# KupynOrest/head_detector

Hardware: AMD Instinct MI355X
Metric: images/sec at 640x640 (VGGHeads forward path: net -> top-k/NMS -> FLAME decode) (higher is better)
Workload: dtype bf16; 1 GPU; vgg_heads_l bf16 batch 64/GPU @ 640x640, u8 NHWC input resident in HBM, ~2.88 heads/img decoded; one step = 8 forwards of that batch back to back (512 images per GPU per step); global_batch=64, image_size=640, parallelism=dp1, graph=False, exchange_to_rank0=False, overlap_post=True, batch_split=2, ramp_steps=30

## Files before the change

### head_detector_amd/csrc/detect.hip

```cpp
#include <hip/hip_runtime.h>

#include <cstring>
#include <new>
#include <vector>

#include "vgh_internal.h"

struct vgh_detector {
    vgh_net* net = nullptr;
    vgh_flame* flame = nullptr;
    vgh_detect_cfg cfg{};
    int device = 0, S = 0, arena_batch = 0, A = 0;
    float* boxes_all = nullptr;
    float* scores_all = nullptr;
    int32_t* idx = nullptr;
    float* cand_scores = nullptr;
    float* cand_boxes = nullptr;
    float* cand_flame = nullptr;
    int32_t* keep_idx = nullptr;
    int32_t* head_row = nullptr;
    int32_t* head_image = nullptr;
    int32_t* ticket = nullptr;
    bool lazy_flame = false;
    enum : uint8_t { SRC_NONE = 0, SRC_EAGER = 1, SRC_LAZY = 2 };
    std::vector<uint8_t> row_src;
    int lazy_rows = 0;
    uint64_t lazy_gen = 0;
    bool overlap = false, side_pending = false;
    hipStream_t side = nullptr, side_main = nullptr;
    bool side_low = true;
    bool side_own = false;
    hipEvent_t ev_net = nullptr, ev_cand = nullptr, ev_side = nullptr;
    vgh_lb_batch* lb = nullptr;
    const float* raw_unpad = nullptr;
};

namespace {

__global__ __launch_bounds__(1024) void head_list_kernel(const int32_t* __restrict__ counts, int B, int keep_k, int capacity, int32_t* __restrict__ head_row,
                                                        int32_t* __restrict__ head_image, int32_t* __restrict__ n_heads) {
    __shared__ int s_off[1025];
    const int t = threadIdx.x;
    const int per = (B + 1023) / 1024;
    const int b0 = t * per, b1 = min(B, b0 + per);
    int mine = 0;
    for (int b = b0; b < b1; ++b) mine += min(max(counts[b], 0), keep_k);
    s_off[t] = mine;
    __syncthreads();
    for (int d = 1; d < 1024; d <<= 1) {
        const int v = (t >= d) ? s_off[t - d] : 0;
        __syncthreads();
        s_off[t] += v;
        __syncthreads();
    }
    int at = s_off[t] - mine;
    if (t == 1023) *n_heads = min(s_off[1023], capacity);
    for (int b = b0; b < b1; ++b) {
        const int c = min(max(counts[b], 0), keep_k);
        for (int i = 0; i < c; ++i) {
            if (at + i < capacity) {
                head_row[at + i] = b * keep_k + i;
                head_image[at + i] = b;
            }
        }
        at += c;
    }
}

constexpr bool kSideLowPriority = true;

void release_side(vgh_detector* d) {
    if (!d->side) return;
    (void)hipStreamSynchronize(d->side);
    if (d->side_own)
        (void)hipStreamDestroy(d->side);
    else
        vgh_stream_release_internal(d->device, d->side, d->side_low);
    d->side = nullptr;
    d->side_own = false;
}

int ensure_side(vgh_detector* d, hipStream_t main) {
    if (d->side && d->side_main == main) return VGH_OK;
    hipStream_t avoid[4] = {main};
    if (int rc = vgh_net_lane_streams(d->net, main, avoid + 1)) return rc;
    release_side(d);
    if (int rc = vgh_stream_acquire_internal(d->device, avoid, 4, &d->side, d->side_low)) return rc;
    d->side_main = main;
    return VGH_OK;
}

}

extern "C" {

int vgh_detector_create(vgh_net* net, vgh_flame* flame, const vgh_detect_cfg* cfg, vgh_detector** out) {
    VGH_REQUIRE(net && cfg && out, "detector_create: null argument");
    VGH_REQUIRE(cfg->n_levels >= 1 && cfg->n_levels <= VGH_MAX_LEVELS, "detector_create: n_levels must be 1..%d", VGH_MAX_LEVELS);
    VGH_REQUIRE(cfg->pre_k >= 1 && cfg->pre_k <= 1024, "detector_create: pre_k must be 1..1024 (vgh_nms limit)");
    VGH_REQUIRE(cfg->keep_k >= 1 && cfg->keep_k <= cfg->pre_k, "detector_create: keep_k must be 1..pre_k");
    VGH_REQUIRE(cfg->max_batch >= 1, "detector_create: max_batch must be positive");
    VGH_REQUIRE(cfg->shape_live >= 0 && cfg->shape_live <= 300 && cfg->expr_live >= 0 && cfg->expr_live <= 100, "detector_create: live counts out of range");
    vgh_detector* d = new (std::nothrow) vgh_detector();
    VGH_REQUIRE(d, "detector_create: out of host memory");
    d->net = net;
    d->flame = flame;
    d->cfg = *cfg;
    d->S = vgh_net_image_size(net);
    d->device = vgh_net_device(net);
    d->arena_batch = vgh_net_max_batch(net);
    int A = 0;
    for (int l = 0; l < cfg->n_levels; ++l) {
        if (!vgh_net_buffer(net, cfg->level_buf[l])) {
            delete d;
            vgh_set_error("detector_create: level %d names buffer %d which the net does not have", l, cfg->level_buf[l]);
            return VGH_ERR_INVALID;
        }
        A += cfg->level_h[l] * cfg->level_w[l];
    }
    d->A = A;
    d->row_src.assign((size_t)cfg->max_batch, vgh_detector::SRC_NONE);
    if (cfg->pre_k > A) {
        delete d;
        vgh_set_error("detector_create: pre_k %d exceeds the %d anchors", cfg->pre_k, A);
        return VGH_ERR_INVALID;
    }
    const size_t MB = (size_t)cfg->max_batch, K = (size_t)cfg->pre_k, KK = (size_t)cfg->keep_k;
#define ALLOC(field, count)                                                           \
    if (hipMalloc((void**)&d->field, (count) * sizeof(*d->field)) != hipSuccess) {     \
        vgh_set_error("detector_create: hipMalloc(%s, %zu) failed", #field, (size_t)((count) * sizeof(*d->field))); \
        vgh_detector_destroy(d);                                                      \
        return VGH_ERR_NOMEM;                                                         \
    }
    ALLOC(boxes_all, MB * A * 4);
    ALLOC(scores_all, MB * A);
    ALLOC(idx, MB * K);
    ALLOC(cand_scores, MB * K);
    ALLOC(cand_boxes, MB * K * 4);
    ALLOC(cand_flame, MB * K * VGH_NUM_FLAME_PARAMS);
    ALLOC(keep_idx, MB * KK);
    ALLOC(head_row, MB * KK);
    ALLOC(head_image, MB * KK);
    ALLOC(ticket, 1);
#undef ALLOC
    if (hipMemset(d->ticket, 0, sizeof(int32_t)) != hipSuccess) {
        vgh_set_error("detector_create: hipMemset failed");
        vgh_detector_destroy(d);
        return VGH_ERR_HIP;
    }
    *out = d;
    return VGH_OK;
}

void vgh_detector_destroy(vgh_detector* d) {
    if (!d) return;
    hipFree(d->boxes_all);
    hipFree(d->scores_all);
    hipFree(d->idx);
    hipFree(d->cand_scores);
    hipFree(d->cand_boxes);
    hipFree(d->cand_flame);
    hipFree(d->keep_idx);
    hipFree(d->head_row);
    hipFree(d->head_image);
    hipFree(d->ticket);
    vgh_lb_destroy(d->lb);
    release_side(d);
    if (d->net) vgh_net_set_pred_guard(d->net, nullptr);
    if (d->ev_net) hipEventDestroy(d->ev_net);
    if (d->ev_cand) hipEventDestroy(d->ev_cand);
    if (d->ev_side) hipEventDestroy(d->ev_side);
    delete d;
}

int vgh_detector_candidates(vgh_detector* d, const void* images_dev, int image_fmt, int B, void* stream) {
    VGH_REQUIRE(d && images_dev, "detector_candidates: null argument");
    VGH_REQUIRE(B >= 1 && B <= d->cfg.max_batch, "detector_candidates: batch %d outside 1..%d", B, d->cfg.max_batch);
    VGH_REQUIRE(image_fmt == VGH_IMG_F32_NCHW || image_fmt == VGH_IMG_U8_NHWC || image_fmt == VGH_IMG_U8_RAW || image_fmt == VGH_IMG_YUV420_RAW,
                "detector_candidates: unknown image format %d", image_fmt);
    const bool raw = image_fmt == VGH_IMG_U8_RAW || image_fmt == VGH_IMG_YUV420_RAW;
    if (raw)
        if (int rc = vgh_lb_prepare(&d->lb, d->S, d->cfg.max_batch, d->arena_batch, image_fmt, images_dev, B)) return rc;
    const int fmt = raw ? VGH_IMG_U8_NHWC : image_fmt;
    const size_t img_bytes = (size_t)d->S * d->S * 3 * (fmt == VGH_IMG_F32_NCHW ? 4 : 1);
    const bool lazy = d->lazy_flame;
    if (B > d->arena_batch) d->lazy_flame = false;
    int rc = VGH_OK;
    for (int at = 0; at < B && !rc; at += d->arena_batch) {
        const int n = (B - at < d->arena_batch) ? B - at : d->arena_batch;
        const void* img = (const char*)images_dev + (size_t)at * img_bytes;
        if (raw) {
            rc = vgh_lb_chunk(d->lb, at / d->arena_batch, n, (hipStream_t)stream);
            img = vgh_lb_canvas(d->lb);
        }
        if (!rc) rc = vgh_net_forward(d->net, img, fmt, n, stream);
        if (!rc) rc = vgh_detector_decode_candidates(d, n, at, stream);
    }
    d->lazy_flame = lazy;
    d->raw_unpad = raw ? vgh_lb_unpad(d->lb) : nullptr;
    return rc;
}

int vgh_detector_decode_candidates(vgh_detector* d, int n, int at, void* stream) {
    VGH_REQUIRE(d, "detector_decode_candidates: null handle");
    VGH_REQUIRE(n >= 1 && at >= 0 && at + n <= d->cfg.max_batch && n <= d->arena_batch, "detector_decode_candidates: rows [%d,%d) outside the buffers", at, at + n);
    const vgh_detect_cfg& c = d->cfg;
    vgh_head_level lv[VGH_MAX_LEVELS];
    for (int l = 0; l < c.n_levels; ++l) {
        lv[l].pred_dev = (const float*)vgh_net_buffer(d->net, c.level_buf[l]);
        lv[l].h = c.level_h[l];
        lv[l].w = c.level_w[l];
        lv[l].pitch = c.level_pitch[l];
        lv[l].stride = c.level_stride[l];
    }
    void* st = stream;
    if (d->overlap) {
        if (int rc0 = ensure_side(d, (hipStream_t)stream)) return rc0;
        VGH_HIP(hipEventRecord(d->ev_net, (hipStream_t)stream));
        VGH_HIP(hipStreamWaitEvent(d->side, d->ev_net, 0));
        st = d->side;
    }
    float* ba = d->boxes_all + (size_t)at * d->A * 4;
    float* sa = d->scores_all + (size_t)at * d->A;
    int32_t* ix = d->idx + (size_t)at * c.pre_k;
    int rc;
    if ((rc = vgh_head_decode(lv, c.n_levels, n, ba, sa, st))) return rc;
    if ((rc = vgh_topk(sa, n, d->A, c.pre_k, ix, d->cand_scores + (size_t)at * c.pre_k, st))) return rc;
    const bool lazy = d->lazy_flame && at == 0;
    if ((rc = vgh_gather_candidates(lv, c.n_levels, n, d->A, c.shape_live, c.expr_live, ba, ix, c.pre_k, d->cand_boxes + (size_t)at * c.pre_k * 4,
                                    lazy ? nullptr : d->cand_flame + (size_t)at * c.pre_k * VGH_NUM_FLAME_PARAMS, st)))
        return rc;
    if (lazy) {
        for (int r = n; r < d->lazy_rows; ++r)
            if (d->row_src[r] == vgh_detector::SRC_LAZY) d->row_src[r] = vgh_detector::SRC_NONE;
        std::memset(d->row_src.data(), vgh_detector::SRC_LAZY, (size_t)n);
        d->lazy_rows = n;
        d->lazy_gen = vgh_net_generation(d->net);
    } else {
        std::memset(d->row_src.data() + at, vgh_detector::SRC_EAGER, (size_t)n);
    }
    if (d->overlap) {
        VGH_HIP(hipEventRecord(d->ev_cand, d->side));
        if ((rc = vgh_net_set_pred_guard(d->net, d->ev_cand))) return rc;
        d->side_pending = true;
    }
    return VGH_OK;
}

int vgh_detector_candidate_buffers(vgh_detector* d, float** boxes_dev, float** scores_dev, float** flame_dev) {
    VGH_REQUIRE(d, "detector_candidate_buffers: null handle");
    if (boxes_dev) *boxes_dev = d->cand_boxes;
    if (scores_dev) *scores_dev = d->cand_scores;
    if (flame_dev) *flame_dev = d->cand_flame;
    return VGH_OK;
}

void* vgh_detector_scratch(vgh_detector* d, int which) {
    if (!d) return nullptr;
    switch (which) {
        case VGH_SCRATCH_BOXES_ALL: return d->boxes_all;
        case VGH_SCRATCH_SCORES_ALL: return d->scores_all;
        case VGH_SCRATCH_TOPK_IDX: return d->idx;
        case VGH_SCRATCH_KEEP_IDX: return d->keep_idx;
        case VGH_SCRATCH_HEAD_ROW: return d->head_row;
        case VGH_SCRATCH_UNPAD: return vgh_lb_unpad(d->lb);
        case VGH_SCRATCH_CANVAS: return vgh_lb_canvas(d->lb);
        default: return nullptr;
    }
}

int vgh_detector_set_flame(vgh_detector* d, vgh_flame* flame) {
    VGH_REQUIRE(d, "detector_set_flame: null handle");
    d->flame = flame;
    return VGH_OK;
}

static int select_on(vgh_detector* d, int B, float conf_thr, float iou_thr, vgh_detect_out* o, void* stream) {
    const vgh_detect_cfg& c = d->cfg;
    int rc;
    const bool want_heads = o->proj_dev || o->verts_dev || o->rot_dev || o->rpy_dev || o->n_heads_dev || o->head_image_dev;
    VGH_REQUIRE(!want_heads || o->n_heads_dev, "detector_select: n_heads_dev is required when any per-head output is requested");
    const int cap_all = B * c.keep_k;
    const int capacity = (o->head_capacity > 0 && o->head_capacity < cap_all) ? o->head_capacity : cap_all;
    int32_t* himg = o->head_image_dev ? o->head_image_dev : d->head_image;
    int n_lazy = 0, n_none = 0;
    for (int r = 0; r < B; ++r) {
        n_lazy += d->row_src[r] == vgh_detector::SRC_LAZY;
        n_none += d->row_src[r] == vgh_detector::SRC_NONE;
    }
    VGH_REQUIRE(n_none == 0, "detector_select: %d of the candidate rows [0,%d) have no valid source (no candidate stage has filled them, or a shorter lazy one replaced theirs)", n_none, B);
    VGH_REQUIRE(n_lazy == 0 || n_lazy == B,
                "detector_select: rows [0,%d) mix %d lazily gathered rows with eagerly gathered ones; decode every chunk of such a batch with the lazy FLAME gather off", B, n_lazy);
    const bool lazy = n_lazy > 0;
    VGH_REQUIRE(!lazy || d->lazy_gen == vgh_net_generation(d->net),
                "detector_select: the candidates were gathered lazily from the predictions of forward %llu, but %llu forward(s) have been queued on the net since: the prediction "
                "buffers no longer hold that batch (queue the select before the next forward, or decode with the lazy FLAME gather off)",
                (unsigned long long)d->lazy_gen, (unsigned long long)(vgh_net_generation(d->net) - d->lazy_gen));
    VGH_REQUIRE(!lazy || c.keep_k <= 1024, "detector_select: the lazy FLAME gather needs keep_k <= 1024");
    if (c.keep_k <= 1024) {
        vgh_head_level lv[VGH_MAX_LEVELS];
        for (int l = 0; l < c.n_levels; ++l) {
            lv[l].pred_dev = (const float*)vgh_net_buffer(d->net, c.level_buf[l]);
            lv[l].h = c.level_h[l];
            lv[l].w = c.level_w[l];
            lv[l].pitch = c.level_pitch[l];
            lv[l].stride = c.level_stride[l];
        }
        if ((rc = vgh_nms_select(d->cand_boxes, d->cand_scores, d->cand_flame, B, c.pre_k, conf_thr, iou_thr, c.keep_k, d->keep_idx, o->counts_dev, o->boxes_dev,
                                 o->scores_dev, o->flame_dev, capacity, want_heads ? d->head_row : nullptr, himg, o->n_heads_dev, d->ticket, lazy ? lv : nullptr,
                                 c.n_levels, lazy ? d->idx : nullptr, c.shape_live, c.expr_live, stream)))
            return rc;
        if (lazy && d->overlap && stream == (void*)d->side) {
            VGH_HIP(hipEventRecord(d->ev_cand, d->side));
        }
        if (!want_heads) return VGH_OK;
    } else {
        if ((rc = vgh_nms(d->cand_boxes, d->cand_scores, B, c.pre_k, conf_thr, iou_thr, c.keep_k, d->keep_idx, o->counts_dev, stream))) return rc;
        if ((rc = vgh_compact(d->cand_boxes, d->cand_scores, d->cand_flame, B, c.pre_k, d->keep_idx, c.keep_k, o->boxes_dev, o->scores_dev, o->flame_dev, stream)))
            return rc;
        if (!want_heads) return VGH_OK;
        hipLaunchKernelGGL(head_list_kernel, dim3(1), dim3(1024), 0, (hipStream_t)stream, (const int32_t*)o->counts_dev, B, c.keep_k, capacity, d->head_row, himg,
                           o->n_heads_dev);
        VGH_HIP(hipGetLastError());
    }
    if (!(o->proj_dev || o->verts_dev || o->rot_dev || o->rpy_dev)) return VGH_OK;
    VGH_REQUIRE(d->flame, "detector_select: per-head FLAME outputs requested but the detector was created without a FLAME handle");
    const float* unpad = o->unpad_dev ? o->unpad_dev : d->raw_unpad;
    if ((rc = vgh_flame_decode_indirect(d->flame, o->flame_dev, d->head_row, himg, o->n_heads_dev, capacity, c.shape_live, c.expr_live, unpad, o->verts_dev,
                                        o->rot_dev, o->rpy_dev, o->proj_dev, stream)))
        return rc;
    return unpad && unpad == d->raw_unpad ? vgh_lb_unpad_read(d->lb, (hipStream_t)stream) : VGH_OK;
}

int vgh_detector_select(vgh_detector* d, int B, float conf_thr, float iou_thr, vgh_detect_out* o, void* stream) {
    VGH_REQUIRE(d && o, "detector_select: null argument");
    VGH_REQUIRE(B >= 1 && B <= d->cfg.max_batch, "detector_select: batch %d outside 1..%d", B, d->cfg.max_batch);
    VGH_REQUIRE(o->boxes_dev && o->scores_dev && o->flame_dev && o->counts_dev, "detector_select: boxes/scores/flame/counts outputs are mandatory");
    if (!d->overlap) return select_on(d, B, conf_thr, iou_thr, o, stream);
    if (int rc0 = ensure_side(d, (hipStream_t)stream)) return rc0;
    const int rc = select_on(d, B, conf_thr, iou_thr, o, d->side);
    d->side_pending = true;
    return rc;
}

#ifdef VGH_EXPERIMENTS
int vgh_detector_set_side_priority(vgh_detector* d, int low) {
    VGH_REQUIRE(d, "detector_set_side_priority: null handle");
    if ((low != 0) == d->side_low) return VGH_OK;
    if (d->side) VGH_HIP(hipStreamSynchronize(d->side));
    release_side(d);
    if (d->net) vgh_net_set_pred_guard(d->net, nullptr);
    d->side_pending = false;
    d->side_low = low != 0;
    return VGH_OK;
}
#endif

int vgh_detector_set_overlap(vgh_detector* d, int enable) {
    VGH_REQUIRE(d, "detector_set_overlap: null handle");
    if (enable && !d->ev_net) {
        VGH_HIP(hipEventCreateWithFlags(&d->ev_net, hipEventDisableTiming));
        VGH_HIP(hipEventCreateWithFlags(&d->ev_cand, hipEventDisableTiming));
        VGH_HIP(hipEventCreateWithFlags(&d->ev_side, hipEventDisableTiming));
    }
    if (!enable && d->side) {
        VGH_HIP(hipStreamSynchronize(d->side));
        vgh_net_set_pred_guard(d->net, nullptr);
        d->side_pending = false;
    }
    d->overlap = enable != 0;
    return VGH_OK;
}

int vgh_detector_set_lazy_flame(vgh_detector* d, int enable) {
    VGH_REQUIRE(d, "detector_set_lazy_flame: null handle");
    d->lazy_flame = enable != 0;
    return VGH_OK;
}

int vgh_detector_streams(vgh_detector* d, void* main_stream, void** out) {
    VGH_REQUIRE(d && out, "detector_streams: null argument");
    hipStream_t lanes[3];
    if (int rc = vgh_net_lane_streams(d->net, (hipStream_t)main_stream, lanes)) return rc;
    for (int i = 0; i < 3; ++i) out[i] = (void*)lanes[i];
    out[3] = nullptr;
    if (d->overlap) {
        if (int rc = ensure_side(d, (hipStream_t)main_stream)) return rc;
        out[3] = (void*)d->side;
    }
    return VGH_OK;
}

int vgh_detector_join(vgh_detector* d, void* stream) {
    VGH_REQUIRE(d, "detector_join: null handle");
    if (d->overlap && d->side && d->side_pending) {
        VGH_HIP(hipEventRecord(d->ev_side, d->side));
        VGH_HIP(hipStreamWaitEvent((hipStream_t)stream, d->ev_side, 0));
    }
    return VGH_OK;
}

int vgh_detector_record(vgh_detector* d, void* event, void* stream) {
    VGH_REQUIRE(d && event, "detector_record: null argument");
    if (d->overlap && d->side && d->side_pending)
        VGH_HIP(hipEventRecord((hipEvent_t)event, d->side));
    else
        VGH_HIP(hipEventRecord((hipEvent_t)event, (hipStream_t)stream));
    return VGH_OK;
}

int vgh_detect(vgh_detector* d, const void* images_dev, int image_fmt, int B, float conf_thr, float iou_thr, vgh_detect_out* o, void* stream) {
    int rc = vgh_detector_candidates(d, images_dev, image_fmt, B, stream);
    if (rc) return rc;
    return vgh_detector_select(d, B, conf_thr, iou_thr, o, stream);
}

}
```

### head_detector_amd/csrc/net.hip

```cpp
#include <stdarg.h>

#include <atomic>
#include <memory>
#include <vector>

#include "net_plan.h"
#include "per_device.h"
#include "vgh_internal.h"

static thread_local char g_err[1024] = "";

void vgh_set_error(const char* fmt, ...) {
    va_list ap;
    va_start(ap, fmt);
    vsnprintf(g_err, sizeof(g_err), fmt, ap);
    va_end(ap);
}

struct NetOp {
    vgh_op_desc d;
    uint16_t* wpack = nullptr;
    float* wf32 = nullptr;
    float* bias = nullptr;
    float out_scale = 1.0f;
    int auto_cfg = -1;
    uint16_t* wds = nullptr;
    float* gscale = nullptr;
    float* dvec = nullptr;
    int overhang_ok = 0, b2b = 0;
    hipEvent_t ev_done = nullptr;
};

static std::atomic<int> g_i8_diag{1};

struct vgh_net {
    int device = 0, image_size = 0, max_batch = 0;
    std::vector<vgh_buf_desc> bufs;
    std::vector<void*> buf_ptr;
    std::vector<int64_t> buf_bytes;
    std::vector<NetOp> ops;
    char* arena = nullptr;
    char* wblob = nullptr;
    uint16_t* zeros = nullptr;
    hipGraph_t graph = nullptr;
    hipGraphExec_t graph_exec = nullptr;
    static constexpr int kLanes = kNetLanes;
    hipStream_t side[kLanes] = {nullptr, nullptr, nullptr, nullptr};
    hipStream_t lanes_main = nullptr;
    bool lanes_ready = false;
    hipEvent_t ev_fork = nullptr, ev_join[kLanes] = {nullptr, nullptr, nullptr, nullptr}, ev_lag[kLanes] = {nullptr, nullptr, nullptr, nullptr};
    hipEvent_t pred_guard = nullptr;
    int nsplit = 1;
    int stem_pair = -1;
    bool lane_wait_cycle = false;
    int fuse_b2b = 1;
    int stem3_ok = 0;
    uint64_t generation = 0;
    int fuse_stem = 0;
};

static inline int64_t buf_image_bytes(const vgh_buf_desc& b) { return (int64_t)b.h * b.w * b.pitch * vgh_fmt_bytes(b.is_f32); }
static inline char* buf_at(const vgh_net* n, int id, int at) { return (char*)n->buf_ptr[id] + at * buf_image_bytes(n->bufs[id]); }

static int net_conv_args(vgh_net* n, const NetOp& op, int B, int at, ConvArgs* a) {
    const vgh_op_desc& d = op.d;
    const vgh_buf_desc &ib = n->bufs[d.in_buf], &ob = n->bufs[d.out_buf];
    const vgh_buf_desc* rb = d.res_buf >= 0 ? &n->bufs[d.res_buf] : nullptr;
    conv_args_fill(a, d, ConvGeom{ib.is_f32, ob.is_f32 == VGH_FMT_F32, vgh_fmt_q8_kind(ob.is_f32), B, ib.h, ib.w, ib.pitch, ob.pitch, rb ? rb->pitch : 0, vgh_fmt_planes(ob.is_f32), rb ? vgh_fmt_planes(rb->is_f32) : 0});
    a->in = (const uint16_t*)buf_at(n, d.in_buf, at);
    a->out = buf_at(n, d.out_buf, at);
    a->res = rb ? (const uint16_t*)buf_at(n, d.res_buf, at) : nullptr;
    a->wpack = op.wpack;
    a->bias = op.bias;
    a->gscale = op.gscale;
    a->dvec = op.dvec;
    a->out_scale = op.out_scale;
    a->zeros = n->zeros;
    const bool in8 = vgh_fmt_is_q8(ib.is_f32), out8 = vgh_fmt_is_q8(ob.is_f32);
    VGH_REQUIRE(a->out_f32 || ob.is_f32 == ib.is_f32 || (in8 && ob.is_f32 == VGH_FMT_BF16) || (out8 && ib.is_f32 == VGH_FMT_BF16), "net: op writes buffer %d in another format than it reads", d.out_buf);
    VGH_REQUIRE(!rb || rb->is_f32 == (in8 ? VGH_FMT_BF16 : ib.is_f32), "net: residual buffer %d has another format than the input", d.res_buf);
    VGH_REQUIRE(!(in8 || out8) || (d.ksize == 3 && d.stride == 1 && !d.grp_cout && !d.shuffle && (!in8 || d.cin % 64 == 0)), "net: an e4m3 buffer can only link plain 3x3 / stride-1 convs (cin %% 64 == 0)");
    const int eh = d.shuffle ? 2 * a->Ho : a->Ho, ew = d.shuffle ? 2 * a->Wo : a->Wo;
    VGH_REQUIRE(ob.h == eh && ob.w == ew, "net: op output buffer %d is %dx%d, conv produces %dx%d", d.out_buf, ob.h, ob.w, eh, ew);
    VGH_REQUIRE(op.overhang_ok || d.in_coff + d.cin + (d.grp_cout ? (d.cout_pad / d.grp_cout - 1) * d.grp_in_stride : 0) <= ib.pitch, "net: conv reads past the input pitch (buf %d)", d.in_buf);
    return VGH_OK;
}

static void net_b2b_fields(ConvArgs& a, const ConvArgs& a2) {
    a.w2pack = a2.wpack;
    a.bias2 = a2.bias;
    a.out2 = a2.out;
    a.out2_pitch = a2.out_pitch;
    a.out2_coff = a2.out_coff;
    a.out2_coff2 = a2.out_coff2;
    a.out2_split = a2.out_split;
    a.cout2_pad = a2.cout_pad;
    a.cout2_store = a2.cout_store;
    a.act2 = a2.act;
}

static bool stem_in_pair_launch(const vgh_net* n) { return n->fuse_b2b == 1 && n->stem_pair >= 0 && n->stem3_ok == 1 && n->ops[n->stem_pair + 1].b2b == 1; }

static int net_run_op(vgh_net* n, const NetOp& op, const void* image0, int fmt, int B, int at, hipStream_t st, int share = 1) {
    const vgh_op_desc& d = op.d;
    const void* image = (const char*)image0 + (int64_t)at * n->image_size * n->image_size * 3 * (fmt == VGH_IMG_F32_NCHW ? 4 : 1);
    const int op_index = (int)(&op - n->ops.data());
    const bool fused = n->fuse_stem && n->stem_pair >= 0;
    const bool stem3 = stem_in_pair_launch(n) && !fused && fmt == VGH_IMG_U8_NHWC;
    switch (d.kind) {
        case VGH_OP_STEM: {
            if (stem3 && op_index == n->stem_pair) {
                const NetOp &ds = n->ops[op_index + 1], &nx = n->ops[op_index + 2];
                ConvArgs a, a2;
                if (int rc = net_conv_args(n, ds, B, at, &a)) return rc;
                if (int rc = net_conv_args(n, nx, B, at, &a2)) return rc;
                a.grid_share = share;
                net_b2b_fields(a, a2);
                return vgh_launch_stem_ds_b2b(a, image, n->image_size, n->image_size, op.wf32, op.bias, st);
            }
#ifdef VGH_EXPERIMENTS
            if (fused && op_index == n->stem_pair) {
                const NetOp& ds = n->ops[op_index + 1];
                const vgh_buf_desc& db = n->bufs[ds.d.out_buf];
                return vgh_launch_stem_ds(image, fmt, B, n->image_size, n->image_size, op.wf32, op.bias, ds.wds, ds.bias, (uint16_t*)buf_at(n, ds.d.out_buf, at), db.pitch, ds.d.out_coff, st);
            }
#endif
            const vgh_buf_desc& ob = n->bufs[d.out_buf];
            if (ob.is_f32 == VGH_FMT_F32)
                return vgh_launch_stem_f32(image, fmt, B, n->image_size, n->image_size, op.wf32, op.bias, (float*)buf_at(n, d.out_buf, at), ob.pitch, d.out_coff, st);
            if (ob.is_f32 == VGH_FMT_F16)
                return vgh_launch_stem(image, fmt, B, n->image_size, n->image_size, op.wf32, op.bias, (uint16_t*)buf_at(n, d.out_buf, at), ob.pitch, d.out_coff, d.cout_store, VGH_FMT_F16X2, 0, st);
            return vgh_launch_stem(image, fmt, B, n->image_size, n->image_size, op.wf32, op.bias, (uint16_t*)buf_at(n, d.out_buf, at), (int64_t)ob.pitch * vgh_fmt_planes(ob.is_f32), d.out_coff,
                                   d.cout_store, ob.is_f32, ob.pitch, st);
        }
        case VGH_OP_CONV: {
            if ((fused || stem3) && op_index == n->stem_pair + 1) return VGH_OK;
            if (n->fuse_b2b && op.b2b == 2) return VGH_OK;
            ConvArgs a;
            if (int rc = net_conv_args(n, op, B, at, &a)) return rc;
            a.grid_share = share;
            if (n->fuse_b2b && op.b2b == 1) {
                const NetOp& nx = n->ops[op_index + 1];
                ConvArgs a2;
                if (int rc = net_conv_args(n, nx, B, at, &a2)) return rc;
                net_b2b_fields(a, a2);
                a.b2b_igemm = n->fuse_b2b == 2;
                return vgh_launch_conv_b2b(a, st);
            }
            if (n->bufs[d.in_buf].is_f32 != VGH_FMT_F32) {
                a.fallback_cfg1 = op.auto_cfg + 1;
                return vgh_launch_conv(a, d.force_cfg >= 0 ? d.force_cfg : op.auto_cfg, st);
            }
            VGH_REQUIRE(a.out_f32 && (d.res_buf < 0 || n->bufs[d.res_buf].is_f32 == VGH_FMT_F32), "net: fp32 conv needs fp32 output / residual buffers");
            VGH_REQUIRE(!d.grp_cout, "net: the fp32 FMA kernel has no grouped mode");
            return vgh_launch_conv_f32(a, op.wf32, st);
        }
        case VGH_OP_SPP_POOL: {
            const vgh_buf_desc& ib = n->bufs[d.in_buf];
            if (ib.is_f32 == VGH_FMT_F32) return vgh_launch_spp_pool_f32((float*)buf_at(n, d.in_buf, at), ib.pitch, d.in_coff, d.cin, B, ib.h, ib.w, st);
            if (ib.is_f32 == VGH_FMT_F16) return vgh_launch_spp_pool((uint16_t*)buf_at(n, d.in_buf, at), ib.pitch, d.in_coff, d.cin, B, ib.h, ib.w, VGH_FMT_F16X2, 0, st);
            return vgh_launch_spp_pool((uint16_t*)buf_at(n, d.in_buf, at), (int64_t)ib.pitch * vgh_fmt_planes(ib.is_f32), d.in_coff, d.cin, B, ib.h, ib.w, ib.is_f32, ib.pitch, st);
        }
        case VGH_OP_FORK:
            return VGH_OK;
        default:
            VGH_REQUIRE(false, "net: unknown op kind %d", d.kind);
    }
    return VGH_OK;
}

static int ensure_lanes(vgh_net* n, hipStream_t main) {
    if (n->lanes_ready && n->lanes_main == main) return VGH_OK;
    hipStreamCaptureStatus cs = hipStreamCaptureStatusNone;
    if (hipStreamIsCapturing(main, &cs) == hipSuccess && cs != hipStreamCaptureStatusNone) {
        VGH_REQUIRE(n->lanes_ready, "net: the lane streams cannot be picked while the caller's stream is capturing; run vgh_net_capture (or one forward) first");
        return VGH_OK;
    }
    hipStream_t avoid[vgh_net::kLanes] = {main};
    for (int l = 1; l < vgh_net::kLanes; ++l) {
        if (n->side[l]) {
            VGH_HIP(hipStreamSynchronize(n->side[l]));
            vgh_stream_release_internal(n->device, n->side[l]);
            n->side[l] = nullptr;
        }
    }
    for (int l = 1; l < vgh_net::kLanes; ++l) {
        if (int rc = vgh_stream_acquire_internal(n->device, avoid, l, &n->side[l])) return rc;
        avoid[l] = n->side[l];
    }
    n->lanes_main = main;
    n->lanes_ready = true;
    return VGH_OK;
}

int vgh_net_lane_streams(vgh_net* n, hipStream_t main, hipStream_t* out) {
    if (int rc = ensure_lanes(n, main)) return rc;
    for (int l = 1; l < vgh_net::kLanes; ++l) out[l - 1] = n->side[l];
    return VGH_OK;
}

static std::atomic<int> g_lane_lag{0};

static int net_forward_split(vgh_net* n, const void* image_dev, int image_fmt, int B, hipStream_t main) {
    const int L = n->nsplit < B ? n->nsplit : B;
    int at[vgh_net::kLanes + 1];
    at[0] = 0;
    for (int l = 0; l < L; ++l) at[l + 1] = at[l] + rows_of_lane(B, L, l);
    VGH_HIP(hipEventRecord(n->ev_fork, main));
    for (int l = 1; l < L; ++l) VGH_HIP(hipStreamWaitEvent(n->side[l], n->ev_fork, 0));
    std::vector<const NetOp*> seq;
    seq.reserve(n->ops.size());
    for (const NetOp& op : n->ops)
        if (op.d.kind != VGH_OP_FORK) seq.push_back(&op);
    const int N = (int)seq.size();
    int lag = g_lane_lag.load(std::memory_order_relaxed);
    if (lag < 0) lag = 0;
    if (lag > N) lag = N;
    bool guard_pending[vgh_net::kLanes];
    for (int l = 0; l < L; ++l) guard_pending[l] = n->pred_guard != nullptr;
    for (int s = 0; s < N + lag * (L - 1); ++s) {
        for (int l = 0; l < L; ++l) {
            const int i = s - l * lag;
            if (i < 0 || i >= N) continue;
            const NetOp& op = *seq[i];
            hipStream_t st = l == 0 ? main : n->side[l];
            if (lag > 0 && l > 0 && i == 0) VGH_HIP(hipStreamWaitEvent(st, n->ev_lag[l - 1], 0));
            if (guard_pending[l] && op.d.kind == VGH_OP_CONV && n->bufs[op.d.out_buf].is_f32 == VGH_FMT_F32) {
                VGH_HIP(hipStreamWaitEvent(st, n->pred_guard, 0));
                guard_pending[l] = false;
            }
            if (int rc = net_run_op(n, op, image_dev, image_fmt, at[l + 1] - at[l], at[l], st)) return rc;
            if (lag > 0 && l + 1 < L && i == lag - 1) VGH_HIP(hipEventRecord(n->ev_lag[l], st));
        }
    }
    for (int l = 1; l < L; ++l) {
        VGH_HIP(hipEventRecord(n->ev_join[l], n->side[l]));
        VGH_HIP(hipStreamWaitEvent(main, n->ev_join[l], 0));
    }
    return VGH_OK;
}

static void pack_weights(const NetPlan& plan, const vgh_buf_desc* bufs, const vgh_op_desc* ops, int n_ops, const float* weights_host, const float* biases_host, char* host, float* oscale) {
#ifdef VGH_EXPERIMENTS
    if (plan.stem_pair >= 0) vgh_pack_stem_ds_weights_host(weights_host + ops[plan.stem_pair + 1].w_off, (uint16_t*)(host + plan.wds));
#endif
    for (int i = 0; i < n_ops; ++i) {
        const vgh_op_desc& d = ops[i];
        const NetPlan::Op& po = plan.ops[i];
        if (d.kind == VGH_OP_CONV) {
            const int wf = bufs[d.in_buf].is_f32;
            if (wf == VGH_FMT_F32)
                memcpy(host + po.w, weights_host + d.w_off, (size_t)d.cout_pad * d.ksize * d.ksize * d.cin * 4);
            else if (wf == VGH_FMT_BF16)
                vgh_pack_conv_weights_host(weights_host + d.w_off, d.cout_pad, d.ksize, d.cin, (uint16_t*)(host + po.w));
            else if (vgh_fmt_is_q8(wf))
                ;
            else
                vgh_pack_conv_weights_split_host(weights_host + d.w_off, d.cout_pad, d.ksize, d.cin, wf, (uint16_t*)(host + po.w), &oscale[i]);
            memcpy(host + po.bias, biases_host + d.b_off, (size_t)d.cout_pad * 4);
            if (po.gscale >= 0) {
                float* g = (float*)(host + po.gscale);
                float* bq = (float*)(host + po.bias);
                const float s_out = vgh_fmt_is_q8(bufs[d.out_buf].is_f32) ? bufs[d.out_buf].scale : 1.0f;
                if (wf == VGH_FMT_I8) {
                    std::vector<float> ws(d.cout_pad);
                    const float* wsrc = weights_host + d.w_off;
                    std::vector<float> peeled;
                    if (po.dvec >= 0) {
                        peeled.assign(wsrc, wsrc + (size_t)d.cout_pad * 9 * d.cin);
                        float* dv = (float*)(host + po.dvec);
                        for (int c = 0; c < d.cout_pad; ++c) {
                            float& wd = peeled[(size_t)c * 9 * d.cin + (size_t)4 * d.cin + c];
                            dv[c] = wd * bufs[d.in_buf].scale;
                            wd = 0.0f;
                        }
                        wsrc = peeled.data();
                    }
                    vgh_pack_conv_weights_i8_host(wsrc, d.cout_pad, d.ksize, d.cin, (uint8_t*)(host + po.w), ws.data());
                    for (int c = 0; c < d.cout_pad; ++c) {
                        const float acc_unit = ws[c] * bufs[d.in_buf].scale;
                        g[c] = acc_unit / s_out;
                        const float bi = __builtin_nearbyintf(bq[c] / acc_unit);
                        const int32_t b32 = bi != bi ? 0 : bi > 2.0e9f ? 2000000000 : bi < -2.0e9f ? -2000000000 : (int32_t)bi;
                        memcpy(&bq[c], &b32, 4);
                    }
                } else if (wf == VGH_FMT_FP8) {
                    std::vector<float> ws(d.cout_pad);
                    vgh_pack_conv_weights_fp8_host(weights_host + d.w_off, d.cout_pad, d.ksize, d.cin, (uint8_t*)(host + po.w), ws.data());
                    for (int c = 0; c < d.cout_pad; ++c) {
                        const float acc_unit = ws[c] * bufs[d.in_buf].scale;
                        bq[c] = bq[c] / acc_unit;
                        g[c] = acc_unit / s_out;
                    }
                } else {
                    for (int c = 0; c < d.cout_pad; ++c) g[c] = 1.0f / s_out;
                }
            }
        } else if (d.kind == VGH_OP_STEM) {
            float* dst = (float*)(host + po.w);
            for (int co = 0; co < 48; ++co)
                for (int k = 0; k < 27; ++k) dst[k * 48 + co] = weights_host[d.w_off + co * 27 + k];
            memcpy(host + po.bias, biases_host + d.b_off, 48 * 4);
        }
    }
}

static int require_canvas(const char* who, int image_fmt) {
    VGH_REQUIRE(image_fmt == VGH_IMG_F32_NCHW || image_fmt == VGH_IMG_U8_NHWC, "%s: image format %d is not a canvas (VGH_IMG_U8_RAW and VGH_IMG_YUV420_RAW are letterboxed by vgh_detect)", who, image_fmt);
    return VGH_OK;
}

struct NetDestroy {
    void operator()(vgh_net* net) const { vgh_net_destroy(net); }
};

extern "C" {

const char* vgh_version(void) { return "vgh 0.1.0 (gfx950)"; }
const char* vgh_last_error(void) { return g_err; }
int vgh_abi_version(void) { return VGH_ABI_VERSION; }

int vgh_net_create(int device, int image_size, int max_batch, const vgh_buf_desc* bufs, int n_bufs, const vgh_op_desc* ops, int n_ops,
                   const float* weights_host, int64_t n_weights, const float* biases_host, int64_t n_biases, vgh_net** out) {
    VGH_REQUIRE(out && bufs && ops && weights_host && biases_host, "net_create: null argument");
    VGH_REQUIRE(max_batch >= 1 && image_size >= 32 && image_size % 32 == 0, "net_create: bad max_batch / image_size");
    NetPlan plan;
    if (int rc = net_plan(image_size, max_batch, bufs, n_bufs, ops, n_ops, weights_host, n_weights, n_biases, g_i8_diag.load(std::memory_order_relaxed) != 0, &plan)) {
        vgh_set_error("%s", plan.err);
        return rc;
    }
    VGH_HIP(hipSetDevice(device));
    std::unique_ptr<vgh_net, NetDestroy> guard(new vgh_net());
    vgh_net* n = guard.get();
    n->device = device;
    n->image_size = image_size;
    n->max_batch = max_batch;
    n->bufs.assign(bufs, bufs + n_bufs);
    n->buf_bytes = plan.buf_bytes;
    n->stem_pair = plan.stem_pair;
    n->lane_wait_cycle = plan.lane_wait_cycle;
    VGH_HIP(hipMalloc((void**)&n->arena, plan.arena_bytes));
    VGH_HIP(hipMemset(n->arena, 0, plan.arena_bytes));
    for (int i = 0; i < n_bufs; ++i) n->buf_ptr.push_back(n->arena + plan.buf_off[i]);
    VGH_HIP(hipMalloc((void**)&n->zeros, 256));
    VGH_HIP(hipMemset(n->zeros, 0, 256));
    VGH_HIP(hipEventCreateWithFlags(&n->ev_fork, hipEventDisableTiming));
    for (int l = 1; l < vgh_net::kLanes; ++l) VGH_HIP(hipEventCreateWithFlags(&n->ev_join[l], hipEventDisableTiming));
    for (int l = 0; l < vgh_net::kLanes; ++l) VGH_HIP(hipEventCreateWithFlags(&n->ev_lag[l], hipEventDisableTiming));
    std::vector<char> host(plan.blob_bytes > 0 ? plan.blob_bytes : 1, 0);
    std::vector<float> oscale(n_ops, 1.0f);
    pack_weights(plan, bufs, ops, n_ops, weights_host, biases_host, host.data(), oscale.data());
    VGH_HIP(hipMalloc((void**)&n->wblob, host.size()));
    VGH_HIP(hipMemcpy(n->wblob, host.data(), host.size(), hipMemcpyHostToDevice));
    for (int i = 0; i < n_ops; ++i) {
        const NetPlan::Op& po = plan.ops[i];
        NetOp op;
        op.d = ops[i];
        op.out_scale = oscale[i];
        op.overhang_ok = po.overhang_ok;
        op.b2b = po.b2b;
        if (ops[i].kind == VGH_OP_CONV || ops[i].kind == VGH_OP_STEM) {
            op.wf32 = (float*)(n->wblob + po.w);
            op.bias = (float*)(n->wblob + po.bias);
        }
        if (ops[i].kind == VGH_OP_CONV) op.wpack = (uint16_t*)(n->wblob + po.w);
        if (po.gscale >= 0) op.gscale = (float*)(n->wblob + po.gscale);
        if (po.dvec >= 0) op.dvec = (float*)(n->wblob + po.dvec);
        if (plan.wds >= 0 && i == plan.stem_pair + 1) op.wds = (uint16_t*)(n->wblob + plan.wds);
        n->ops.push_back(op);
        if (po.ev_done) VGH_HIP(hipEventCreateWithFlags(&n->ops[i].ev_done, hipEventDisableTiming));
    }
    for (NetOp& op : n->ops) {
        if (op.d.kind != VGH_OP_CONV || n->bufs[op.d.in_buf].is_f32 == VGH_FMT_F32) continue;
        ConvArgs ref;
        if (int rc = net_conv_args(n, op, n->max_batch, 0, &ref)) return rc;
        if (int rc = vgh_conv_prepare(ref)) return rc;
        op.auto_cfg = vgh_conv_pick_auto(ref);
    }
    if (n->stem_pair >= 0 && n->stem_pair + 2 < (int)n->ops.size() && n->ops[n->stem_pair + 1].b2b == 1 && image_size % 32 == 0) {
        ConvArgs a, a2;
        if (!net_conv_args(n, n->ops[n->stem_pair + 1], 1, 0, &a) && !net_conv_args(n, n->ops[n->stem_pair + 2], 1, 0, &a2)) {
            net_b2b_fields(a, a2);
            if (!vgh_conv_prepare(a)) n->stem3_ok = vgh_conv_ds_b2b_ok(a) && a.act == VGH_ACT_RELU ? 1 : 0;
        }
    }
    *out = guard.release();
    return VGH_OK;
}

void vgh_net_destroy(vgh_net* n) {
    if (!n) return;
    if (n->graph_exec) hipGraphExecDestroy(n->graph_exec);
    if (n->graph) hipGraphDestroy(n->graph);
    for (int l = 1; l < vgh_net::kLanes; ++l) {
        if (n->side[l]) {
            hipStreamSynchronize(n->side[l]);
            vgh_stream_release_internal(n->device, n->side[l]);
        }
        if (n->ev_join[l]) hipEventDestroy(n->ev_join[l]);
    }
    for (int l = 0; l < vgh_net::kLanes; ++l)
        if (n->ev_lag[l]) hipEventDestroy(n->ev_lag[l]);
    if (n->ev_fork) hipEventDestroy(n->ev_fork);
    for (NetOp& op : n->ops)
        if (op.ev_done) hipEventDestroy(op.ev_done);
    hipFree(n->arena);
    hipFree(n->wblob);
    hipFree(n->zeros);
    delete n;
}

int vgh_net_forward(vgh_net* n, const void* image_dev, int image_fmt, int B, void* stream) {
    VGH_REQUIRE(n && image_dev, "net_forward: null argument");
    if (int rc = require_canvas("net_forward", image_fmt)) return rc;
    VGH_REQUIRE(B >= 0 && B <= n->max_batch, "net_forward: B=%d exceeds max_batch=%d", B, n->max_batch);
    hipStream_t main = (hipStream_t)stream;
    ++n->generation;
    if (int rc = ensure_lanes(n, main)) return rc;
    if (n->nsplit > 1 && B > 1) return net_forward_split(n, image_dev, image_fmt, B, main);
    bool pending[vgh_net::kLanes] = {false, false, false, false}, used[vgh_net::kLanes] = {false, false, false, false};
    bool guard_pending = n->pred_guard != nullptr;
    for (const NetOp& op : n->ops) {
        if (guard_pending && op.d.kind == VGH_OP_CONV && n->bufs[op.d.out_buf].is_f32 == VGH_FMT_F32) {
            VGH_HIP(hipStreamWaitEvent(main, n->pred_guard, 0));
            for (int l = 1; l < vgh_net::kLanes; ++l)
                if (n->side[l]) VGH_HIP(hipStreamWaitEvent(n->side[l], n->pred_guard, 0));
            guard_pending = false;
        }
        if (op.d.kind == VGH_OP_FORK) {
            VGH_HIP(hipEventRecord(n->ev_fork, main));
            for (int l = 1; l < vgh_net::kLanes; ++l) pending[l] = true;
            continue;
        }
        const int lane_f = op.d.lane & 0xff, dep = (op.d.lane >> 8) - 1;
        const int lane = (lane_f > 0 && lane_f < vgh_net::kLanes) ? lane_f : 0;
        hipStream_t st = main;
        if (lane > 0) {
            st = n->side[lane];
            if (pending[lane]) {
                VGH_HIP(hipStreamWaitEvent(st, n->ev_fork, 0));
                pending[lane] = false;
            }
            used[lane] = true;
        }
        if (dep >= 0 && dep < (int)n->ops.size() && n->ops[dep].ev_done) VGH_HIP(hipStreamWaitEvent(st, n->ops[dep].ev_done, 0));
        if (int rc = net_run_op(n, op, image_dev, image_fmt, B, 0, st)) return rc;
        if (op.ev_done) VGH_HIP(hipEventRecord(op.ev_done, st));
    }
    for (int l = 1; l < vgh_net::kLanes; ++l)
        if (used[l]) {
            VGH_HIP(hipEventRecord(n->ev_join[l], n->side[l]));
            VGH_HIP(hipStreamWaitEvent(main, n->ev_join[l], 0));
        }
    return VGH_OK;
}

int vgh_net_profile(vgh_net* n, const void* image_dev, int image_fmt, int B, void* stream, float* op_ms) {
    VGH_REQUIRE(n && image_dev && op_ms, "net_profile: null argument");
    if (int rc = require_canvas("net_profile", image_fmt)) return rc;
    VGH_REQUIRE(B >= 0 && B <= n->max_batch, "net_profile: B=%d exceeds max_batch=%d", B, n->max_batch);
    hipStream_t st = (hipStream_t)stream;
    ++n->generation;
    if (int rc = ensure_lanes(n, st)) return rc;
    const size_t m = n->ops.size();
    struct Events {
        std::vector<hipEvent_t> v;
        ~Events() {
            for (hipEvent_t e : v)
                if (e) hipEventDestroy(e);
        }
    } events{std::vector<hipEvent_t>(m + 1, nullptr)};
    std::vector<hipEvent_t>& ev = events.v;
    for (auto& e : ev) VGH_HIP(hipEventCreate(&e));
    VGH_HIP(hipEventRecord(ev[0], st));
    const int L = (n->nsplit > 1 && B > 1) ? (n->nsplit < B ? n->nsplit : B) : 1;
    for (size_t i = 0; i < m; ++i) {
        if (L == 1) {
            if (int rc = net_run_op(n, n->ops[i], image_dev, image_fmt, B, 0, st)) return rc;
        } else {
            VGH_HIP(hipEventRecord(n->ev_fork, st));
            int at = 0;
            for (int l = 0; l < L; ++l) {
                const int nb = rows_of_lane(B, L, l);
                hipStream_t ls = l == 0 ? st : n->side[l];
                if (l > 0) VGH_HIP(hipStreamWaitEvent(ls, n->ev_fork, 0));
                if (int rc = net_run_op(n, n->ops[i], image_dev, image_fmt, nb, at, ls)) return rc;
                if (l > 0) {
                    VGH_HIP(hipEventRecord(n->ev_join[l], ls));
                    VGH_HIP(hipStreamWaitEvent(st, n->ev_join[l], 0));
                }
                at += nb;
            }
        }
        VGH_HIP(hipEventRecord(ev[i + 1], st));
    }
    VGH_HIP(hipEventSynchronize(ev[m]));
    for (size_t i = 0; i < m; ++i) VGH_HIP(hipEventElapsedTime(&op_ms[i], ev[i], ev[i + 1]));
    return VGH_OK;
}

int vgh_net_capture(vgh_net* n, const void* image_dev, int image_fmt, int B, void* stream) {
    VGH_REQUIRE(n && stream, "net_capture: needs a non-null stream");
    if (int rc = require_canvas("net_capture", image_fmt)) return rc;
    VGH_REQUIRE(!n->pred_guard, "net_capture: a prediction guard event is set (detector overlap mode); graph replay cannot honour it");
    VGH_REQUIRE(!n->lane_wait_cycle, "net_capture: two side lanes of this program wait for each other's ops; the HIP runtime cannot end the capture of such a program (run it eagerly, "
                "or lay the lanes out so that the wait-for relation among lanes 1..3 is acyclic, as arch.schedule_latency does)");
    hipStream_t st = (hipStream_t)stream;
    if (n->graph_exec) {
        hipGraphExecDestroy(n->graph_exec);
        n->graph_exec = nullptr;
    }
    if (n->graph) {
        hipGraphDestroy(n->graph);
        n->graph = nullptr;
    }
    if (int rc = ensure_lanes(n, st)) return rc;
    VGH_HIP(hipStreamBeginCapture(st, hipStreamCaptureModeThreadLocal));
    int rc = vgh_net_forward(n, image_dev, image_fmt, B, stream);
    hipError_t e = hipStreamEndCapture(st, &n->graph);
    if (rc) return rc;
    VGH_HIP(e);
    VGH_HIP(hipGraphInstantiate(&n->graph_exec, n->graph, nullptr, nullptr, 0));
    return VGH_OK;
}

int vgh_net_forward_graph(vgh_net* n, void* stream) {
    VGH_REQUIRE(n && n->graph_exec, "net_forward_graph: call vgh_net_capture first");
    VGH_REQUIRE(!n->pred_guard, "net_forward_graph: a prediction guard event is set (detector overlap mode); use vgh_net_forward");
    ++n->generation;
    VGH_HIP(hipGraphLaunch(n->graph_exec, (hipStream_t)stream));
    return VGH_OK;
}

void* vgh_net_buffer(vgh_net* n, int buf_id) { return (n && buf_id >= 0 && buf_id < (int)n->buf_ptr.size()) ? n->buf_ptr[buf_id] : nullptr; }
int64_t vgh_net_buffer_bytes(vgh_net* n, int buf_id) { return (n && buf_id >= 0 && buf_id < (int)n->buf_bytes.size()) ? n->buf_bytes[buf_id] : -1; }

#ifdef VGH_EXPERIMENTS
int vgh_net_set_lane_lag(int ops) {
    VGH_REQUIRE(ops >= 0, "net_set_lane_lag: negative");
    g_lane_lag.store(ops, std::memory_order_relaxed);
    return VGH_OK;
}
#endif

int vgh_net_set_split(vgh_net* n, int nsplit) {
    VGH_REQUIRE(n, "net_set_split: null handle");
    VGH_REQUIRE(nsplit >= 1 && nsplit <= vgh_net::kLanes, "net_set_split: 1..%d lanes", vgh_net::kLanes);
    n->nsplit = nsplit;
    return VGH_OK;
}

#ifdef VGH_EXPERIMENTS
int vgh_net_set_fuse_stem(vgh_net* n, int enable) {
    VGH_REQUIRE(n, "net_set_fuse_stem: null handle");
    n->fuse_stem = enable ? 1 : 0;
    return VGH_OK;
}
#endif

int vgh_net_set_pred_guard(vgh_net* n, void* event) {
    VGH_REQUIRE(n, "net_set_pred_guard: null handle");
    n->pred_guard = (hipEvent_t)event;
    return VGH_OK;
}

int vgh_net_set_b2b(vgh_net* n, int enable) {
    VGH_REQUIRE(n, "net_set_b2b: null handle");
    n->fuse_b2b = (enable == 2 || enable == 3) ? enable : enable ? 1 : 0;
    return VGH_OK;
}
int vgh_net_stem_fused(vgh_net* n) {
    return n && stem_in_pair_launch(n) ? 1 : 0;
}
int vgh_net_b2b_pairs(vgh_net* n) {
    int k = 0;
    if (n)
        for (const NetOp& op : n->ops) k += op.b2b == 1;
    return k;
}

uint64_t vgh_net_generation(vgh_net* n) { return n ? n->generation : 0; }
int vgh_net_max_batch(vgh_net* n) { return n ? n->max_batch : 0; }
int vgh_net_device(vgh_net* n) { return n ? n->device : 0; }
int vgh_net_image_size(vgh_net* n) { return n ? n->image_size : 0; }

int vgh_net_set_cfg(vgh_net* n, int op_index, int cfg) {
    VGH_REQUIRE(n && op_index >= 0 && op_index < (int)n->ops.size(), "net_set_cfg: bad op index");
    const int fmt0 = n->bufs[n->ops[op_index].d.kind == VGH_OP_CONV ? n->ops[op_index].d.in_buf : 0].is_f32;
    const bool split_net = vgh_fmt_planes(fmt0) > 1 || fmt0 == VGH_FMT_F16;
    VGH_REQUIRE(cfg >= -1 && cfg < (split_net ? vgh_conv_split_num_cfgs() : vgh_conv_num_cfgs()), "net_set_cfg: bad cfg");
    NetOp& op = n->ops[op_index];
    if (cfg >= 0 && op.d.kind == VGH_OP_CONV && !split_net && (n->bufs[op.d.in_buf].is_f32 == VGH_FMT_BF16 || vgh_fmt_is_q8(n->bufs[op.d.in_buf].is_f32))) {
        ConvArgs ref;
        int rc = net_conv_args(n, op, n->max_batch, 0, &ref);
        if (!rc) rc = vgh_conv_prepare(ref);
        if (rc) return rc;
        if (!vgh_conv_cfg_ok_for(cfg, ref)) {
            fprintf(stderr, "[vgh] net_set_cfg: op %d: tile %s cannot run this op at max_batch=%d; its automatic tile %s runs it at every batch size\n", op_index, vgh_conv_cfg_name(cfg),
                    n->max_batch, vgh_conv_cfg_name(op.auto_cfg));
            cfg = -1;
        }
    }
    op.d.force_cfg = cfg;
    return VGH_OK;
}

int vgh_net_op_cfg(vgh_net* n, int op_index) {
    if (!n || op_index < 0 || op_index >= (int)n->ops.size()) return -1;
    const NetOp& op = n->ops[op_index];
    if (op.d.kind != VGH_OP_CONV || n->bufs[op.d.in_buf].is_f32 == VGH_FMT_F32) return -1;
    return op.d.force_cfg >= 0 ? op.d.force_cfg : op.auto_cfg;
}

static uint16_t* g_zeros[kMaxDevices];
static PerDevice g_zeros_made;

int vgh_conv2d(const vgh_conv_call* c, void* stream) {
    VGH_REQUIRE(c && c->in_dev && c->wpack_dev && c->bias_dev && c->out_dev, "conv2d: null argument");
    int dev = 0;
    VGH_HIP(hipGetDevice(&dev));
    VGH_REQUIRE(device_slot(hipSuccess, dev) != kNoSlot, "conv2d: device index");
    hipError_t zeros_err = hipSuccess;
    once_per_device(g_zeros_made, dev, [&] {
        uint16_t* z = nullptr;
        if ((zeros_err = hipMalloc((void**)&z, 256)) == hipSuccess && (zeros_err = hipMemset(z, 0, 256)) == hipSuccess) g_zeros[dev] = z;
        return zeros_err == hipSuccess ? 1 : 0;
    });
    VGH_HIP(zeros_err);
    VGH_REQUIRE(c->fmt == VGH_FMT_BF16 || c->fmt == VGH_FMT_BF16X2 || c->fmt == VGH_FMT_F16X2 || c->fmt == VGH_FMT_FP8 || c->fmt == VGH_FMT_F16 || c->fmt == VGH_FMT_I8, "conv2d: fmt %d", c->fmt);
    const int in_fp8 = vgh_fmt_q8_kind(c->fmt);
    VGH_REQUIRE(c->out_fp8 >= 0 && c->out_fp8 <= 2 && (!in_fp8 || !c->out_fp8 || in_fp8 == c->out_fp8), "conv2d: out_fp8 is 0, 1 (e4m3) or 2 (int8), and an 8-bit input keeps its format");
    VGH_REQUIRE(!c->diag_dev || (c->fmt == VGH_FMT_I8 && !c->out_fp8 && c->cin >= c->cout_pad && c->cout_pad <= 1024), "conv2d: diag_dev belongs to an int8 -> bf16 conv with cout_pad <= min(cin, 1024)");
    VGH_REQUIRE(!(in_fp8 || c->out_fp8) || (c->gscale_dev && (vgh_fmt_is_q8(c->fmt) || c->fmt == VGH_FMT_BF16) && !c->out_f32), "conv2d: an e4m3 / int8 conv needs gscale_dev, a bf16 or e4m3 input and no fp32 output");
    const int planes = vgh_fmt_planes(c->fmt);
    ConvArgs a;
    conv_args_fill(&a, *c, ConvGeom{c->fmt, c->out_f32, c->out_fp8, c->B, c->H, c->W, c->in_pitch, c->out_pitch, c->res_pitch, c->out_f32 ? 1 : planes, planes});
    a.in = (const uint16_t*)c->in_dev;
    a.out = c->out_dev;
    a.res = (const uint16_t*)c->res_dev;
    a.wpack = (const uint16_t*)c->wpack_dev;
    a.bias = c->bias_dev;
    a.gscale = c->gscale_dev;
    a.dvec = c->diag_dev;
    a.out_scale = c->out_scale;
    a.zeros = g_zeros[dev];
    return vgh_launch_conv(a, c->force_cfg, (hipStream_t)stream);
}

int vgh_pack_conv_weights(const float* w_host, int cout_pad, int ksize, int cin, uint16_t* wpack_host) {
    VGH_REQUIRE(w_host && wpack_host, "pack: null argument");
    VGH_REQUIRE(cin % 32 == 0 && cout_pad % 32 == 0 && (ksize == 1 || ksize == 3), "pack: cin/cout_pad must be multiples of 32, ksize 1 or 3");
    vgh_pack_conv_weights_host(w_host, cout_pad, ksize, cin, wpack_host);
    return VGH_OK;
}

int vgh_pack_conv_weights_fp8(const float* w_host, int cout_pad, int ksize, int cin, uint8_t* wpack_host, float* wscale_host) {
    VGH_REQUIRE(w_host && wpack_host && wscale_host, "pack_fp8: null argument");
    VGH_REQUIRE(cin % 64 == 0 && cout_pad % 32 == 0 && ksize == 3, "pack_fp8: cin must be a multiple of 64, cout_pad of 32, ksize 3");
    vgh_pack_conv_weights_fp8_host(w_host, cout_pad, ksize, cin, wpack_host, wscale_host);
    return VGH_OK;
}
int vgh_net_set_i8_diag(int on) {
    g_i8_diag.store(on ? 1 : 0, std::memory_order_relaxed);
    return VGH_OK;
}
int vgh_net_op_has_diag(vgh_net* n, int op_index) { return (n && op_index >= 0 && op_index < (int)n->ops.size() && n->ops[op_index].dvec) ? 1 : 0; }
int vgh_pack_conv_weights_i8(const float* w_host, int cout_pad, int ksize, int cin, uint8_t* wpack_host, float* wscale_host) {
    VGH_REQUIRE(w_host && wpack_host && wscale_host, "pack_i8: null argument");
    VGH_REQUIRE(cin % 64 == 0 && cout_pad % 32 == 0 && ksize == 3, "pack_i8: cin must be a multiple of 64, cout_pad of 32, ksize 3");
    vgh_pack_conv_weights_i8_host(w_host, cout_pad, ksize, cin, wpack_host, wscale_host);
    return VGH_OK;
}

int vgh_stream_create(int device, void** stream_out) {
    VGH_REQUIRE(stream_out, "stream_create: null");
    VGH_HIP(hipSetDevice(device));
    hipStream_t s;
    VGH_HIP(hipStreamCreateWithFlags(&s, hipStreamNonBlocking));
    *stream_out = (void*)s;
    return VGH_OK;
}
int vgh_stream_destroy(void* stream) {
    VGH_HIP(hipStreamDestroy((hipStream_t)stream));
    return VGH_OK;
}
int vgh_stream_sync(void* stream) {
    VGH_HIP(hipStreamSynchronize((hipStream_t)stream));
    return VGH_OK;
}
int vgh_event_create(void** ev_out) {
    VGH_REQUIRE(ev_out, "event_create: null");
    hipEvent_t e;
    VGH_HIP(hipEventCreate(&e));
    *ev_out = (void*)e;
    return VGH_OK;
}
int vgh_event_destroy(void* ev) {
    VGH_HIP(hipEventDestroy((hipEvent_t)ev));
    return VGH_OK;
}
int vgh_event_record(void* ev, void* stream) {
    VGH_HIP(hipEventRecord((hipEvent_t)ev, (hipStream_t)stream));
    return VGH_OK;
}
int vgh_event_elapsed_ms(void* ev_start, void* ev_stop, float* ms_out) {
    VGH_REQUIRE(ms_out, "event_elapsed: null");
    VGH_HIP(hipEventSynchronize((hipEvent_t)ev_stop));
    VGH_HIP(hipEventElapsedTime(ms_out, (hipEvent_t)ev_start, (hipEvent_t)ev_stop));
    return VGH_OK;
}

}
```

### head_detector_amd/csrc/net_plan.h

```cpp
#pragma once
#include <math.h>
#include <stdint.h>
#include <stdio.h>
#include <string.h>

#include <vector>

#include "../../include/vgh.h"
#include "conv_tiles.h"

constexpr int kNetLanes = 4;

inline int64_t align_up(int64_t x, int64_t a) { return (x + a - 1) / a * a; }

inline int rows_of_lane(int B, int L, int l) { return B / L + (l < B % L ? 1 : 0); }

struct ConvGeom {
    int fmt;
    int out_f32, out_fp8;
    int B, H, W;
    int64_t in_pitch, out_pitch, res_pitch;
    int out_planes, res_planes;
};
template <class Desc>
inline void conv_args_fill(ConvArgs* a, const Desc& d, const ConvGeom& g) {
    memset(a, 0, sizeof(*a));
    const bool h16 = g.fmt == VGH_FMT_F16;
    a->split = h16 ? VGH_FMT_F16X2 : vgh_fmt_planes(g.fmt) > 1 ? g.fmt : 0;
    a->nseg = h16 ? 1 : 3;
    a->in_plane = h16 ? 0 : (int)g.in_pitch;
    a->out_plane = h16 ? 0 : (int)g.out_pitch;
    a->res_plane = h16 ? 0 : (int)g.res_pitch;
    a->grp_cout = d.grp_cout;
    a->grp_in_stride = d.grp_in_stride;
    a->in_pitch = g.in_pitch * vgh_fmt_planes(g.fmt);
    a->in_coff = d.in_coff;
    a->cin = d.cin;
    a->B = g.B;
    a->H = g.H;
    a->W = g.W;
    a->ksize = d.ksize;
    a->stride = d.stride;
    a->pad = d.ksize / 2;
    a->Ho = (g.H + 2 * a->pad - d.ksize) / d.stride + 1;
    a->Wo = (g.W + 2 * a->pad - d.ksize) / d.stride + 1;
    a->out_pitch = g.out_pitch * g.out_planes;
    a->out_coff = d.out_coff;
    a->out_coff2 = d.out_coff2;
    a->out_split = d.out_split;
    a->cout_pad = d.cout_pad;
    a->cout_store = d.cout_store;
    a->out_f32 = g.out_f32;
    a->res_pitch = g.res_pitch * g.res_planes;
    a->res_coff = d.res_coff;
    a->in_fp8 = vgh_fmt_q8_kind(g.fmt);
    a->out_fp8 = g.out_fp8;
    a->alpha = d.alpha;
    a->act = d.act;
    a->shuffle = d.shuffle;
    a->shuffle_c = d.shuffle ? d.cout_pad / 4 : 0;
    a->P = g.B * a->Ho * a->Wo;
    a->cblocks = d.cin / (a->in_fp8 ? 64 : 32);
    a->nkb = d.ksize * d.ksize * a->cblocks;
}

inline bool i8_peel_diag(const float* w, const vgh_op_desc& d, bool enabled) {
    if (!enabled || d.ksize != 3 || d.stride != 1 || d.grp_cout || d.cin < d.cout_pad || d.cout_pad > 1024) return false;
    const size_t row = (size_t)9 * d.cin;
    int live = 0, dom = 0;
    for (int c = 0; c < d.cout_pad; ++c) {
        float mx = 0.0f;
        for (size_t i = 0; i < row; ++i) mx = fmaxf(mx, fabsf(w[(size_t)c * row + i]));
        if (mx > 0.0f) {
            ++live;
            if (fabsf(w[(size_t)c * row + (size_t)4 * d.cin + c]) >= mx) ++dom;
        }
    }
    return live > 0 && 2 * dom >= live;
}

inline bool sole_link(const vgh_op_desc* ops, int n_ops, int i, int buf) {
    for (int j = 0; j < n_ops; ++j)
        if (j != i && j != i + 1 && (ops[j].kind == VGH_OP_CONV || ops[j].kind == VGH_OP_SPP_POOL) && (ops[j].in_buf == buf || ops[j].out_buf == buf || ops[j].res_buf == buf)) return false;
    return true;
}

struct NetPlan {
    std::vector<int64_t> buf_off, buf_bytes;
    int64_t arena_bytes = 0;
    struct Op {
        int64_t w = 0, bias = 0;
        int64_t gscale = -1;
        int64_t dvec = -1;
        int b2b = 0;
        int overhang_ok = 0;
        int ev_done = 0;
    };
    std::vector<Op> ops;
    int64_t wds = -1;
    int64_t blob_bytes = 0;
    int stem_pair = -1;
    bool lane_wait_cycle = false;
    char err[256] = "";
};

inline int net_plan(int image_size, int max_batch, const vgh_buf_desc* bufs, int n_bufs, const vgh_op_desc* ops, int n_ops, const float* weights, int64_t n_weights, int64_t n_biases,
                    bool i8_diag, NetPlan* p) {
#define PLAN_REQUIRE(cond, ...)                          \
    do {                                                 \
        if (!(cond)) {                                   \
            snprintf(p->err, sizeof(p->err), __VA_ARGS__); \
            return VGH_ERR_INVALID;                      \
        }                                                \
    } while (0)
    *p = NetPlan();
    PLAN_REQUIRE(n_bufs >= 0 && n_ops >= 0, "net_create: negative buffer or op count");
    for (int i = 0; i < n_bufs; ++i) {
        PLAN_REQUIRE(bufs[i].is_f32 >= VGH_FMT_BF16 && bufs[i].is_f32 <= VGH_FMT_I8, "net_create: buffer %d has unknown format %d", i, bufs[i].is_f32);
        PLAN_REQUIRE(!vgh_fmt_is_q8(bufs[i].is_f32) || (bufs[i].scale > 0.0f && bufs[i].scale < 1e30f && bufs[i].pitch % 16 == 0), "net_create: 8-bit buffer %d needs a positive scale and a pitch that is a multiple of 16", i);
        const int64_t bytes = (int64_t)max_batch * bufs[i].h * bufs[i].w * bufs[i].pitch * vgh_fmt_bytes(bufs[i].is_f32);
        p->buf_off.push_back(p->arena_bytes);
        p->buf_bytes.push_back(bytes);
        p->arena_bytes += align_up(bytes + 256, 256);
    }
    const auto buf_ok = [&](int id) { return id >= 0 && id < n_bufs; };
    p->ops.assign(n_ops, NetPlan::Op());
    int64_t at = 0;
    const auto take = [&](int64_t bytes) {
        const int64_t off = at;
        at += align_up(bytes, 256);
        return off;
    };
    for (int i = 0; i < n_ops; ++i) {
        const vgh_op_desc& d = ops[i];
        NetPlan::Op& o = p->ops[i];
        if (d.kind == VGH_OP_CONV) {
            PLAN_REQUIRE(d.cin % 32 == 0 && d.cout_pad % 32 == 0, "net_create: op %d channel padding", i);
            PLAN_REQUIRE(buf_ok(d.in_buf) && buf_ok(d.out_buf) && d.res_buf < n_bufs, "net_create: op %d buffer ids", i);
            const int64_t we = (int64_t)d.cout_pad * d.ksize * d.ksize * d.cin;
            PLAN_REQUIRE(d.w_off >= 0 && d.w_off + we <= n_weights && d.b_off >= 0 && d.b_off + d.cout_pad <= n_biases, "net_create: op %d weight range", i);
            const vgh_buf_desc& ib = bufs[d.in_buf];
            if (d.in_coff + d.cin > ib.pitch && !d.grp_cout) {
                const int live = ib.pitch - d.in_coff;
                PLAN_REQUIRE(live > 0 && ib.is_f32 == VGH_FMT_BF16, "net_create: op %d reads past the pitch of buffer %d", i, d.in_buf);
                const float* w = weights + d.w_off;
                for (int64_t r = 0; r < (int64_t)d.cout_pad * d.ksize * d.ksize; ++r)
                    for (int c = live; c < d.cin; ++c)
                        PLAN_REQUIRE(w[r * d.cin + c] == 0.0f, "net_create: op %d reads %d channels of a %d-channel pitch with a non-zero weight at input channel %d", i, d.cin, ib.pitch, c);
                o.overhang_ok = 1;
            }
            const int wf = ib.is_f32, of = bufs[d.out_buf].is_f32;
            o.w = take(we * (vgh_fmt_is_q8(wf) ? 1 : (wf == VGH_FMT_BF16 || wf == VGH_FMT_F16) ? 2 : wf == VGH_FMT_F32 ? 4 : 6));
            o.bias = take((int64_t)d.cout_pad * 4);
            if (vgh_fmt_is_q8(wf) || vgh_fmt_is_q8(of)) {
                o.gscale = take((int64_t)d.cout_pad * 4);
                if (wf == VGH_FMT_I8 && of == VGH_FMT_BF16 && i8_peel_diag(weights + d.w_off, d, i8_diag)) o.dvec = take((int64_t)d.cout_pad * 4);
            }
        } else if (d.kind == VGH_OP_STEM) {
            PLAN_REQUIRE(buf_ok(d.out_buf), "net_create: op %d buffer ids", i);
            PLAN_REQUIRE(d.w_off >= 0 && d.w_off + 27 * 48 <= n_weights && d.b_off >= 0 && d.b_off + 48 <= n_biases, "net_create: stem weight range");
            o.w = take(27 * 48 * 4);
            o.bias = take(64 * 4);
        } else if (d.kind == VGH_OP_SPP_POOL) {
            PLAN_REQUIRE(buf_ok(d.in_buf), "net_create: op %d buffer ids", i);
        }
        if (d.lane >> 8) {
            const int dep = (d.lane >> 8) - 1;
            PLAN_REQUIRE(dep >= 0 && dep < i, "net_create: op %d waits for op %d, which does not precede it", i, dep);
            p->ops[dep].ev_done = 1;
        }
    }
    for (int i = 0; i + 1 < n_ops; ++i) {
        const vgh_op_desc &a = ops[i], &d = ops[i + 1];
        if (a.kind != VGH_OP_STEM || d.kind != VGH_OP_CONV) continue;
        if (image_size % 4 == 0  && d.in_buf == a.out_buf && d.in_coff == a.out_coff && d.ksize == 3 && d.stride == 2 && d.cin == 64 &&
            d.cout_pad == 96 && d.cout_store == 96 && d.res_buf < 0 && !d.shuffle && d.out_split >= 96 && d.act == VGH_ACT_RELU && d.grp_cout == 0 && bufs[a.out_buf].is_f32 == VGH_FMT_BF16 &&
            bufs[d.out_buf].is_f32 == VGH_FMT_BF16 && d.out_coff % 8 == 0 && bufs[d.out_buf].pitch % 8 == 0 && sole_link(ops, n_ops, i, a.out_buf)) {
            p->stem_pair = i;
#ifdef VGH_EXPERIMENTS
            p->wds = take((int64_t)9 * 3 * 96 * 16 * 2);
#endif
        }
        break;
    }
    p->blob_bytes = at;
    for (int i = 0; i + 1 < n_ops; ++i) {
        const vgh_op_desc &a = ops[i], &b = ops[i + 1];
        if (a.kind != VGH_OP_CONV || b.kind != VGH_OP_CONV || p->ops[i].b2b != 0) continue;
        const vgh_buf_desc &ab = bufs[a.out_buf], &ai = bufs[a.in_buf], &bo = bufs[b.out_buf];
        if (ab.is_f32 == VGH_FMT_BF16 && ai.is_f32 == VGH_FMT_BF16 && bo.is_f32 == VGH_FMT_BF16 && vgh_conv_b2b_ok(a.ksize, a.stride, a.cout_pad, b.cout_pad) && a.cout_store == a.cout_pad &&
            a.out_coff == 0 && a.out_split >= a.cout_pad && ab.pitch == a.cout_pad && a.res_buf < 0 && !a.shuffle && !a.grp_cout && a.act != VGH_ACT_SILU && b.ksize == 1 && b.stride == 1 &&
            b.in_buf == a.out_buf && b.in_coff == 0 && b.cin == a.cout_pad && b.res_buf < 0 && !b.shuffle && !b.grp_cout && b.act != VGH_ACT_SILU && b.out_coff % 8 == 0 && b.out_coff2 % 8 == 0 &&
            b.out_split % 8 == 0 && b.cout_store % 8 == 0 && bo.pitch % 8 == 0 && sole_link(ops, n_ops, i, a.out_buf)) {
            p->ops[i].b2b = 1;
            p->ops[i + 1].b2b = 2;
        }
    }
    bool w[kNetLanes][kNetLanes] = {};
    for (int i = 0; i < n_ops; ++i) {
        if (!(ops[i].lane >> 8)) continue;
        const int a = ops[i].lane & 0xff, b = ops[(ops[i].lane >> 8) - 1].lane & 0xff;
        if (a > 0 && a < kNetLanes && b > 0 && b < kNetLanes && a != b) w[a][b] = true;
    }
    for (int k = 1; k < kNetLanes; ++k)
        for (int a = 1; a < kNetLanes; ++a)
            for (int b = 1; b < kNetLanes; ++b) w[a][b] = w[a][b] || (w[a][k] && w[k][b]);
    for (int a = 1; a < kNetLanes; ++a) p->lane_wait_cycle = p->lane_wait_cycle || w[a][a];
    return VGH_OK;
#undef PLAN_REQUIRE
}
```

### head_detector_amd/csrc/postproc.hip

```cpp
#include "vgh_internal.h"

namespace {

constexpr int MAX_LEVELS = 4;
struct Levels {
    const float* pred[MAX_LEVELS];
    int h[MAX_LEVELS], w[MAX_LEVELS], pitch[MAX_LEVELS], stride[MAX_LEVELS], start[MAX_LEVELS + 1];
    int n;
};

__device__ __forceinline__ int find_level(const Levels& L, int a) {
    int l = 0;
#pragma unroll
    for (int i = 1; i < MAX_LEVELS; ++i)
        if (i < L.n && a >= L.start[i]) l = i;
    return l;
}

__global__ __launch_bounds__(256) void head_decode_kernel(Levels L, int B, int A, float* __restrict__ boxes, float* __restrict__ scores) {
    const int64_t gid = (int64_t)blockIdx.x * blockDim.x + threadIdx.x;
    if (gid >= (int64_t)B * A) return;
    const int b = (int)(gid / A), a = (int)(gid - (int64_t)b * A);
    const int l = find_level(L, a);
    const int p = a - L.start[l];
    const int hw = L.h[l] * L.w[l];
    const float* pr = L.pred[l] + ((int64_t)b * hw + p) * L.pitch[l];
    const int ay = p / L.w[l], ax = p - ay * L.w[l];
    float d[4];
#pragma unroll
    for (int side = 0; side < 4; ++side) {
        float x[17];
        float m = -INFINITY;
#pragma unroll
        for (int k = 0; k < 17; ++k) {
            x[k] = pr[side * 17 + k];
            m = fmaxf(m, x[k]);
        }
        float s = 0.0f;
#pragma unroll
        for (int k = 0; k < 17; ++k) {
            x[k] = expf(x[k] - m);
            s += x[k];
        }
        float e = 0.0f;
#pragma unroll
        for (int k = 0; k < 17; ++k) e += (x[k] / s) * (float)k;
        d[side] = e;
    }
    const float cx = (float)ax + 0.5f, cy = (float)ay + 0.5f, st = (float)L.stride[l];
    float4 o;
    o.x = (cx - d[0]) * st;
    o.y = (cy - d[1]) * st;
    o.z = (cx + d[2]) * st;
    o.w = (cy + d[3]) * st;
    *(float4*)(boxes + gid * 4) = o;
    scores[gid] = 1.0f / (1.0f + expf(-pr[VGH_PRED_CLS_OFF]));
}

__device__ __forceinline__ uint32_t float_key(float f) {
    uint32_t u = __float_as_uint(f);
    if ((u & 0x7fffffffu) > 0x7f800000u) return 0xffffffffu;
    if (u == 0x80000000u) u = 0u;
    return (u & 0x80000000u) ? ~u : (u | 0x80000000u);
}
template <bool FILTER>
__device__ __forceinline__ uint64_t composite(float f, int idx, float conf) {
    const uint32_t key = (FILTER && !(f >= conf)) ? 0u : float_key(f);
    return ((uint64_t)key << 32) | (uint32_t)(~(uint32_t)idx);
}

template <bool CACHED, bool FILTER>
__global__ __launch_bounds__(1024) void topk_kernel(const float* __restrict__ scores, int A, int k, int32_t* __restrict__ out_idx,
                                                    float* __restrict__ out_scores, float conf) {
    constexpr int RC = 9;
    __shared__ uint32_t hist[256];
    __shared__ uint64_t s_prefix;
    __shared__ int s_kk;
    __shared__ int s_count;
    __shared__ int s_done;
    __shared__ uint64_t sel[1024];
    const int b = blockIdx.x, tid = threadIdx.x;
    const float* sc = scores + (int64_t)b * A;
    if (tid == 0) {
        s_prefix = 0;
        s_kk = k;
        s_count = 0;
        s_done = 0;
    }
    sel[tid] = 0;
    uint64_t cache[RC];
    if constexpr (CACHED) {
#pragma unroll
        for (int r = 0; r < RC; ++r) {
            const int i = tid + r * 1024;
            cache[r] = i < A ? composite<FILTER>(sc[i], i, conf) : 0ull;
        }
    }
    __syncthreads();
    for (int pass = 0; pass < 8; ++pass) {
        const int shift = 56 - 8 * pass;
        if (tid < 256) hist[tid] = 0;
        __syncthreads();
        const uint64_t prefix = s_prefix;
        if constexpr (CACHED) {
#pragma unroll
            for (int r = 0; r < RC; ++r) {
                const uint64_t c = cache[r];
                const bool match = c != 0ull && ((pass == 0) || ((c >> (shift + 8)) == (prefix >> (shift + 8))));
                if (match) atomicAdd(&hist[(c >> shift) & 255], 1u);
            }
        } else {
            for (int i = tid; i < A; i += 1024) {
                const uint64_t c = composite<FILTER>(sc[i], i, conf);
                const bool match = (pass == 0) || ((c >> (shift + 8)) == (prefix >> (shift + 8)));
                if (match) atomicAdd(&hist[(c >> shift) & 255], 1u);
            }
        }
        __syncthreads();
        const int kk = s_kk;
        __syncthreads();
        if (tid < 256) {
            uint32_t above = 0;
            for (int j = tid + 1; j < 256; ++j) above += hist[j];
            const uint32_t mine = hist[tid];
            if ((int)above < kk && kk <= (int)(above + mine)) {
                s_prefix = prefix | ((uint64_t)tid << shift);
                s_kk = kk - (int)above;
                if (kk == (int)(above + mine)) s_done = 1;
            }
        }
        __syncthreads();
        if (s_done) break;
    }
    const uint64_t T = s_prefix;
    if constexpr (CACHED) {
#pragma unroll
        for (int r = 0; r < RC; ++r) {
            const uint64_t c = cache[r];
            if (c != 0ull && c >= T) {
                const int slot = atomicAdd(&s_count, 1);
                if (slot < 1024) sel[slot] = c;
            }
        }
    } else {
        for (int i = tid; i < A; i += 1024) {
            const uint64_t c = composite<FILTER>(sc[i], i, conf);
            if (c >= T) {
                const int slot = atomicAdd(&s_count, 1);
                if (slot < 1024) sel[slot] = c;
            }
        }
    }
    __syncthreads();
    uint64_t v = sel[tid];
    for (int size = 2; size <= 1024; size <<= 1) {
        const bool desc = (tid & size) == 0;
        for (int stride = size >> 1; stride > 0; stride >>= 1) {
            uint64_t pv;
            if (stride >= 64) {
                __syncthreads();
                sel[tid] = v;
                __syncthreads();
                pv = sel[tid ^ stride];
            } else {
                pv = __shfl_xor(v, stride, 64);
            }
            const bool take_max = ((tid & stride) == 0) == desc;
            v = take_max ? (v > pv ? v : pv) : (v < pv ? v : pv);
        }
    }
    if (tid < k) {
        const int idx = (int)(~(uint32_t)(v & 0xffffffffu));
        out_idx[(int64_t)b * k + tid] = idx;
        if (out_scores) out_scores[(int64_t)b * k + tid] = sc[idx];
    }
}

__device__ __forceinline__ float flame_channel(const float* __restrict__ pr, int c, int S, int E, int ax, int ay, float st) {
    const int o_shape = VGH_PRED_FLAME_OFF, o_expr = o_shape + S, o_rot = o_expr + E, o_jaw = o_rot + 6, o_tr = o_jaw + 3, o_sc = o_tr + 3;
    float v = 0.0f;
    if (c < 300) {
        if (c < S) v = tanhf(pr[o_shape + c]) * 3.0f;
    } else if (c < 400) {
        if (c - 300 < E) v = tanhf(pr[o_expr + c - 300]) * 3.0f;
    } else if (c < 403) {
        v = pr[o_rot + 3 + (c - 400)];
    } else if (c < 406) {
        v = pr[o_jaw + (c - 403)];
    } else if (c < 409) {
        v = pr[o_rot + (c - 406)];
    } else if (c == 409) {
        v = pr[o_tr + 0] + ((float)ax + 0.5f) * st;
    } else if (c == 410) {
        v = pr[o_tr + 1] + ((float)ay + 0.5f) * st;
    } else if (c == 411) {
        v = pr[o_tr + 2];
    } else {
        v = (expf(pr[o_sc]) / 0.05f) * st;
    }
    return v;
}

__global__ __launch_bounds__(256) void gather_kernel(Levels L, int A, int S, int E, const float* __restrict__ boxes, const int32_t* __restrict__ idx,
                                                     int k, float* __restrict__ out_boxes, float* __restrict__ out_flame) {
    const int j = blockIdx.x * 4 + (threadIdx.x >> 6), b = blockIdx.y, lane = threadIdx.x & 63;
    if (j >= k) return;
    const int a = idx[(int64_t)b * k + j];
    const int l = find_level(L, a);
    const int p = a - L.start[l];
    const int hw = L.h[l] * L.w[l];
    const float* pr = L.pred[l] + ((int64_t)b * hw + p) * L.pitch[l];
    const int ay = p / L.w[l], ax = p - ay * L.w[l];
    const float st = (float)L.stride[l];
    if (lane < 4) out_boxes[((int64_t)b * k + j) * 4 + lane] = boxes[((int64_t)b * A + a) * 4 + lane];
    if (!out_flame) return;
    float* of = out_flame + ((int64_t)b * k + j) * VGH_NUM_FLAME_PARAMS;
    for (int c = lane; c < VGH_NUM_FLAME_PARAMS; c += 64) of[c] = flame_channel(pr, c, S, E, ax, ay, st);
}

__device__ __forceinline__ bool iou_gt(const float4 a, const float area_a, const float4 b, const float thr) {
#pragma clang fp contract(off)
    const float area_b = (b.z - b.x) * (b.w - b.y);
    const float xx1 = fmaxf(a.x, b.x), yy1 = fmaxf(a.y, b.y);
    const float xx2 = fminf(a.z, b.z), yy2 = fminf(a.w, b.w);
    const float w = fmaxf(0.0f, xx2 - xx1), h = fmaxf(0.0f, yy2 - yy1);
    const float inter = w * h;
    const float ovr = inter / (area_a + area_b - inter);
    return ovr > thr;
}

__device__ __forceinline__ int greedy_nms(const float* __restrict__ boxes, const float* __restrict__ scores, int n_in, float conf, float thr, int keep_k,
                                          int32_t* __restrict__ keep_row, float4* sb, unsigned long long* removed, int* s_keep) {
    const int tid = threadIdx.x;
    bool valid = false;
    if (tid < n_in) {
        sb[tid] = *(const float4*)(boxes + (int64_t)tid * 4);
        valid = scores[tid] >= conf;
    }
    const unsigned long long bal = __ballot(valid);
    if ((tid & 63) == 0) removed[tid >> 6] = ~bal;
    for (int j = tid; j < keep_k; j += 1024) keep_row[j] = -1;
    __syncthreads();
    int kept = 0;
    int i = 0;
    while (kept < keep_k) {
        int nxt = -1;
        for (int wd = i >> 6; wd < 16 && nxt < 0; ++wd) {
            unsigned long long free_bits = ~removed[wd];
            if (wd == (i >> 6)) free_bits &= ~0ull << (i & 63);
            if (free_bits) nxt = wd * 64 + __ffsll((long long)free_bits) - 1;
        }
        if (nxt < 0) break;
        i = nxt;
        if (tid == 0) {
            keep_row[kept] = i;
            if (s_keep) s_keep[kept] = i;
        }
        ++kept;
        const float4 bi = sb[i];
        float area_i;
        {
#pragma clang fp contract(off)
            area_i = (bi.z - bi.x) * (bi.w - bi.y);
        }
        const bool sup = (tid > i) && valid && iou_gt(bi, area_i, sb[valid ? tid : 0], thr);
        const unsigned long long m = __ballot(sup);
        __syncthreads();
        if ((tid & 63) == 0 && m) removed[tid >> 6] |= m;
        __syncthreads();
        ++i;
    }
    return kept;
}

__global__ __launch_bounds__(1024) void nms_kernel(const float* __restrict__ boxes, const float* __restrict__ scores, int n_in, float conf, float thr,
                                                   int keep_k, int32_t* __restrict__ keep_idx, int32_t* __restrict__ counts) {
    __shared__ float4 sb[1024];
    __shared__ unsigned long long removed[16];
    const int b = blockIdx.x;
    const int kept = greedy_nms(boxes + (int64_t)b * n_in * 4, scores + (int64_t)b * n_in, n_in, conf, thr, keep_k, keep_idx + (int64_t)b * keep_k, sb, removed, nullptr);
    if (threadIdx.x == 0) counts[b] = kept;
}

__global__ __launch_bounds__(1024) void nms_select_kernel(const float* __restrict__ boxes, const float* __restrict__ scores, const float* __restrict__ flame, int n_in,
                                                          float conf, float thr, int keep_k, int32_t* __restrict__ keep_idx, int32_t* __restrict__ counts,
                                                          float* __restrict__ ob, float* __restrict__ os, float* __restrict__ of, int B, int capacity,
                                                          int32_t* __restrict__ head_row, int32_t* __restrict__ head_image, int32_t* __restrict__ n_heads,
                                                          int32_t* __restrict__ ticket, Levels L, const int32_t* __restrict__ lazy_idx, int S, int E) {
    __shared__ float4 sb[1024];
    __shared__ unsigned long long removed[16];
    __shared__ int s_keep[1024];
    __shared__ int s_off[1025];
    __shared__ int s_last;
    const int b = blockIdx.x, tid = threadIdx.x;
    const int kept = greedy_nms(boxes + (int64_t)b * n_in * 4, scores + (int64_t)b * n_in, n_in, conf, thr, keep_k, keep_idx + (int64_t)b * keep_k, sb, removed, s_keep);
    if (tid == 0) counts[b] = kept;
    __syncthreads();
    const int w = tid >> 6, lane = tid & 63;
    for (int j = w; j < keep_k; j += 16) {
        const int64_t o = (int64_t)b * keep_k + j;
        if (j >= kept) {
            if (lane < 4) ob[o * 4 + lane] = 0.0f;
            if (lane == 0) os[o] = 0.0f;
            if (of)
                for (int c = lane; c < VGH_NUM_FLAME_PARAMS; c += 64) of[o * VGH_NUM_FLAME_PARAMS + c] = 0.0f;
            continue;
        }
        const int64_t sr = (int64_t)b * n_in + s_keep[j];
        if (lane < 4) ob[o * 4 + lane] = boxes[sr * 4 + lane];
        if (lane == 0) os[o] = scores[sr];
        if (of) {
            if (lazy_idx) {
                const int a = lazy_idx[sr];
                const int l = find_level(L, a);
                const int p = a - L.start[l];
                const float* pr = L.pred[l] + ((int64_t)b * (L.h[l] * L.w[l]) + p) * L.pitch[l];
                const int ay = p / L.w[l], ax = p - ay * L.w[l];
                const float st = (float)L.stride[l];
                for (int c = lane; c < VGH_NUM_FLAME_PARAMS; c += 64) of[o * VGH_NUM_FLAME_PARAMS + c] = flame_channel(pr, c, S, E, ax, ay, st);
            } else {
                for (int c = lane; c < VGH_NUM_FLAME_PARAMS; c += 64) of[o * VGH_NUM_FLAME_PARAMS + c] = flame[sr * VGH_NUM_FLAME_PARAMS + c];
            }
        }
    }
    if (!head_row) return;
    __threadfence();
    __syncthreads();
    if (tid == 0) s_last = (atomicAdd(ticket, 1) == B - 1) ? 1 : 0;
    __syncthreads();
    if (!s_last) return;
    if (tid == 0) *ticket = 0;
    __threadfence();
    const int per = (B + 1023) / 1024;
    const int b0 = tid * per, b1 = min(B, b0 + per);
    int mine = 0;
    for (int q = b0; q < b1; ++q) mine += min(max(__hip_atomic_load(counts + q, __ATOMIC_RELAXED, __HIP_MEMORY_SCOPE_AGENT), 0), keep_k);
    s_off[tid] = mine;
    __syncthreads();
    for (int d = 1; d < 1024; d <<= 1) {
        const int v = (tid >= d) ? s_off[tid - d] : 0;
        __syncthreads();
        s_off[tid] += v;
        __syncthreads();
    }
    int at = s_off[tid] - mine;
    if (tid == 1023) *n_heads = min(s_off[1023], capacity);
    for (int q = b0; q < b1; ++q) {
        const int c = min(max(__hip_atomic_load(counts + q, __ATOMIC_RELAXED, __HIP_MEMORY_SCOPE_AGENT), 0), keep_k);
        for (int e = 0; e < c; ++e) {
            if (at + e < capacity) {
                head_row[at + e] = q * keep_k + e;
                head_image[at + e] = q;
            }
        }
        at += c;
    }
}

__global__ __launch_bounds__(64) void compact_kernel(const float* __restrict__ boxes, const float* __restrict__ scores, const float* __restrict__ flame,
                                                     int n_in, const int32_t* __restrict__ keep_idx, int keep_k, float* __restrict__ ob,
                                                     float* __restrict__ os, float* __restrict__ of) {
    const int j = blockIdx.x, b = blockIdx.y, lane = threadIdx.x;
    const int src = keep_idx[(int64_t)b * keep_k + j];
    const int64_t o = (int64_t)b * keep_k + j;
    if (src < 0) {
        if (lane < 4) ob[o * 4 + lane] = 0.0f;
        if (lane == 0) os[o] = 0.0f;
        if (of)
            for (int c = lane; c < VGH_NUM_FLAME_PARAMS; c += 64) of[o * VGH_NUM_FLAME_PARAMS + c] = 0.0f;
        return;
    }
    const int64_t s = (int64_t)b * n_in + src;
    if (lane < 4) ob[o * 4 + lane] = boxes[s * 4 + lane];
    if (lane == 0) os[o] = scores[s];
    if (of)
        for (int c = lane; c < VGH_NUM_FLAME_PARAMS; c += 64) of[o * VGH_NUM_FLAME_PARAMS + c] = flame[s * VGH_NUM_FLAME_PARAMS + c];
}

__global__ __launch_bounds__(256) void gather_boxes_kernel(const float* __restrict__ boxes, const int32_t* __restrict__ idx, int n, int k, float* __restrict__ out) {
    const int j = blockIdx.x * 256 + threadIdx.x, b = blockIdx.y;
    if (j >= k) return;
    const int src = idx[(int64_t)b * k + j];
    const f32x4_t v = *(const f32x4_t*)(boxes + ((int64_t)b * n + src) * 4);
    *(f32x4_t*)(out + ((int64_t)b * k + j) * 4) = v;
}

__global__ __launch_bounds__(64) void compact_indirect_kernel(const float* __restrict__ boxes, const float* __restrict__ flame, int flame_w, int n,
                                                              const int32_t* __restrict__ idx, const float* __restrict__ sorted_scores, int k,
                                                              const int32_t* __restrict__ keep_idx, int keep_k, float* __restrict__ ob, float* __restrict__ os,
                                                              float* __restrict__ of) {
    const int j = blockIdx.x, b = blockIdx.y, lane = threadIdx.x;
    const int pos = keep_idx[(int64_t)b * keep_k + j];
    const int64_t o = (int64_t)b * keep_k + j;
    if (pos < 0) {
        if (lane < 4) ob[o * 4 + lane] = 0.0f;
        if (lane == 0) os[o] = 0.0f;
        if (of)
            for (int c = lane; c < flame_w; c += 64) of[o * flame_w + c] = 0.0f;
        return;
    }
    const int64_t s = (int64_t)b * n + idx[(int64_t)b * k + pos];
    if (lane < 4) ob[o * 4 + lane] = boxes[s * 4 + lane];
    if (lane == 0) os[o] = sorted_scores[(int64_t)b * k + pos];
    if (of)
        for (int c = lane; c < flame_w; c += 64) of[o * flame_w + c] = flame[s * flame_w + c];
}

int make_levels(const vgh_head_level* levels, int n_levels, Levels* L) {
    VGH_REQUIRE(n_levels >= 1 && n_levels <= MAX_LEVELS, "head: n_levels=%d out of range", n_levels);
    L->n = n_levels;
    L->start[0] = 0;
    for (int i = 0; i < MAX_LEVELS; ++i) {
        if (i < n_levels) {
            L->pred[i] = levels[i].pred_dev;
            L->h[i] = levels[i].h;
            L->w[i] = levels[i].w;
            L->pitch[i] = levels[i].pitch;
            L->stride[i] = levels[i].stride;
            L->start[i + 1] = L->start[i] + levels[i].h * levels[i].w;
        } else {
            L->pred[i] = nullptr;
            L->h[i] = L->w[i] = L->pitch[i] = L->stride[i] = 0;
            L->start[i + 1] = L->start[i];
        }
    }
    return VGH_OK;
}

template <bool FILTER>
int topk_launch(const float* scores_dev, int B, int A, int k, int32_t* idx_dev, float* topk_scores_dev, float conf, void* stream) {
    VGH_REQUIRE(k >= 1 && k <= 1024, "topk: k=%d must be in [1,1024]", k);
    VGH_REQUIRE(k <= A, "topk: k=%d exceeds the number of anchors %d (torch.topk raises too)", k, A);
    if (B == 0) return VGH_OK;
    if (A <= 9 * 1024)
        hipLaunchKernelGGL((topk_kernel<true, FILTER>), dim3(B), dim3(1024), 0, (hipStream_t)stream, scores_dev, A, k, idx_dev, topk_scores_dev, conf);
    else
        hipLaunchKernelGGL((topk_kernel<false, FILTER>), dim3(B), dim3(1024), 0, (hipStream_t)stream, scores_dev, A, k, idx_dev, topk_scores_dev, conf);
    VGH_HIP(hipGetLastError());
    return VGH_OK;
}

}

extern "C" {

int vgh_head_decode(const vgh_head_level* levels, int n_levels, int B, float* boxes_dev, float* scores_dev, void* stream) {
    Levels L;
    if (int rc = make_levels(levels, n_levels, &L)) return rc;
    const int A = L.start[n_levels];
    if (B * (int64_t)A == 0) return VGH_OK;
    for (int i = 0; i < n_levels; ++i) VGH_REQUIRE(levels[i].pitch >= 69, "head_decode: pitch too small");
    const int64_t total = (int64_t)B * A;
    hipLaunchKernelGGL(head_decode_kernel, dim3((unsigned)((total + 255) / 256)), dim3(256), 0, (hipStream_t)stream, L, B, A, boxes_dev, scores_dev);
    VGH_HIP(hipGetLastError());
    return VGH_OK;
}

int vgh_topk(const float* scores_dev, int B, int A, int k, int32_t* idx_dev, float* topk_scores_dev, void* stream) {
    return topk_launch<false>(scores_dev, B, A, k, idx_dev, topk_scores_dev, 0.0f, stream);
}

int vgh_gather_candidates(const vgh_head_level* levels, int n_levels, int B, int A, int shape_c, int expr_c, const float* boxes_dev,
                          const int32_t* idx_dev, int k, float* out_boxes_dev, float* out_flame_dev, void* stream) {
    Levels L;
    if (int rc = make_levels(levels, n_levels, &L)) return rc;
    VGH_REQUIRE(A == L.start[n_levels], "gather: A=%d does not match the levels (%d)", A, L.start[n_levels]);
    VGH_REQUIRE(shape_c >= 0 && shape_c <= 300 && expr_c >= 0 && expr_c <= 100, "gather: bad live channel counts");
    for (int i = 0; i < n_levels; ++i) VGH_REQUIRE(levels[i].pitch >= VGH_PRED_FLAME_OFF + shape_c + expr_c + 13, "gather: pitch too small");
    if (B == 0 || k == 0) return VGH_OK;
    hipLaunchKernelGGL(gather_kernel, dim3((k + 3) / 4, B), dim3(256), 0, (hipStream_t)stream, L, A, shape_c, expr_c, boxes_dev, idx_dev, k, out_boxes_dev,
                       out_flame_dev);
    VGH_HIP(hipGetLastError());
    return VGH_OK;
}

int vgh_nms(const float* boxes_dev, const float* scores_dev, int B, int n_in, float conf_thr, float iou_thr, int keep_k, int32_t* keep_idx_dev,
            int32_t* counts_dev, void* stream) {
    VGH_REQUIRE(n_in >= 0 && n_in <= 1024, "nms: n_in=%d must be <= 1024", n_in);
    VGH_REQUIRE(keep_k >= 1, "nms: keep_k must be positive");
    if (B == 0) return VGH_OK;
    hipLaunchKernelGGL(nms_kernel, dim3(B), dim3(1024), 0, (hipStream_t)stream, boxes_dev, scores_dev, n_in, conf_thr, iou_thr, keep_k, keep_idx_dev,
                       counts_dev);
    VGH_HIP(hipGetLastError());
    return VGH_OK;
}

}
int vgh_nms_select(const float* boxes_dev, const float* scores_dev, const float* flame_dev, int B, int n_in, float conf_thr, float iou_thr, int keep_k,
                   int32_t* keep_idx_dev, int32_t* counts_dev, float* out_boxes_dev, float* out_scores_dev, float* out_flame_dev, int capacity, int32_t* head_row_dev,
                   int32_t* head_image_dev, int32_t* n_heads_dev, int32_t* ticket_dev, const vgh_head_level* lazy_levels, int n_levels, const int32_t* lazy_idx_dev,
                   int shape_c, int expr_c, void* stream) {
    VGH_REQUIRE(n_in >= 0 && n_in <= 1024 && keep_k >= 1 && keep_k <= 1024, "nms_select: n_in=%d / keep_k=%d must be <= 1024", n_in, keep_k);
    VGH_REQUIRE(!head_row_dev || (head_image_dev && n_heads_dev && ticket_dev), "nms_select: the head list needs head_image, n_heads and the ticket");
    if (B == 0) return VGH_OK;
    Levels L;
    memset(&L, 0, sizeof(L));
    if (lazy_idx_dev) {
        VGH_REQUIRE(lazy_levels, "nms_select: the lazy FLAME gather needs the head levels");
        if (int rc = make_levels(lazy_levels, n_levels, &L)) return rc;
    }
    hipLaunchKernelGGL(nms_select_kernel, dim3(B), dim3(1024), 0, (hipStream_t)stream, boxes_dev, scores_dev, flame_dev, n_in, conf_thr, iou_thr, keep_k, keep_idx_dev,
                       counts_dev, out_boxes_dev, out_scores_dev, out_flame_dev, B, capacity, head_row_dev, head_image_dev, n_heads_dev, ticket_dev, L, lazy_idx_dev, shape_c,
                       expr_c);
    VGH_HIP(hipGetLastError());
    return VGH_OK;
}

extern "C" {
int vgh_compact(const float* boxes_dev, const float* scores_dev, const float* flame_dev, int B, int n_in, const int32_t* keep_idx_dev, int keep_k,
                float* out_boxes_dev, float* out_scores_dev, float* out_flame_dev, void* stream) {
    if (B == 0) return VGH_OK;
    hipLaunchKernelGGL(compact_kernel, dim3(keep_k, B), dim3(64), 0, (hipStream_t)stream, boxes_dev, scores_dev, flame_dev, n_in, keep_idx_dev, keep_k,
                       out_boxes_dev, out_scores_dev, out_flame_dev);
    VGH_HIP(hipGetLastError());
    return VGH_OK;
}

int64_t vgh_topk_nms_workspace_bytes(int B, int n, int pre_k, int keep_k) {
    const int64_t k = pre_k < n ? pre_k : n;
    return (int64_t)B * (k * 4  + k * 4  + k * 16  + (int64_t)keep_k * 4 ) + 256;
}

int vgh_topk_nms(const float* boxes_dev, const float* scores_dev, const float* flame_dev, int flame_width, int B, int n, float conf_thr, float iou_thr, int pre_k,
                 int keep_k, void* workspace_dev, float* out_boxes_dev, float* out_scores_dev, float* out_flame_dev, int32_t* counts_dev, void* stream) {
    VGH_REQUIRE(boxes_dev && scores_dev && workspace_dev && out_boxes_dev && out_scores_dev && counts_dev, "topk_nms: null argument");
    VGH_REQUIRE((flame_dev == nullptr) == (out_flame_dev == nullptr) && (!flame_dev || flame_width > 0), "topk_nms: flame input / output must both be given or both be NULL");
    VGH_REQUIRE(B >= 0 && n >= 1 && pre_k >= 1 && keep_k >= 1, "topk_nms: bad sizes");
    const int k = pre_k < n ? pre_k : n;
    VGH_REQUIRE(k <= 1024, "topk_nms: min(pre_k, n) = %d exceeds the 1024 candidates the NMS kernel holds", k);
    if (B == 0) return VGH_OK;
    VGH_REQUIRE(((uintptr_t)workspace_dev & 15) == 0, "topk_nms: workspace must be 16-byte aligned");
    auto al16 = [](size_t x) { return (x + 15) & ~(size_t)15; };
    char* ws = (char*)workspace_dev;
    const size_t o_ssc = al16((size_t)B * k * 4), o_sbx = al16(o_ssc + (size_t)B * k * 4), o_keep = o_sbx + (size_t)B * k * 16;
    int32_t* idx = (int32_t*)ws;
    float* ssc = (float*)(ws + o_ssc);
    float* sbx = (float*)(ws + o_sbx);
    int32_t* keep = (int32_t*)(ws + o_keep);
    int rc;
    if ((rc = topk_launch<true>(scores_dev, B, n, k, idx, ssc, conf_thr, stream))) return rc;
    hipLaunchKernelGGL(gather_boxes_kernel, dim3((k + 255) / 256, B), dim3(256), 0, (hipStream_t)stream, boxes_dev, (const int32_t*)idx, n, k, sbx);
    VGH_HIP(hipGetLastError());
    if ((rc = vgh_nms(sbx, ssc, B, k, conf_thr, iou_thr, keep_k, keep, counts_dev, stream))) return rc;
    hipLaunchKernelGGL(compact_indirect_kernel, dim3(keep_k, B), dim3(64), 0, (hipStream_t)stream, boxes_dev, flame_dev, flame_width, n, (const int32_t*)idx,
                       (const float*)ssc, k, (const int32_t*)keep, keep_k, out_boxes_dev, out_scores_dev, out_flame_dev);
    VGH_HIP(hipGetLastError());
    return VGH_OK;
}

}
```

### head_detector_amd/csrc/vgh_internal.h

```cpp
#pragma once
#include <hip/hip_runtime.h>
#include <stdint.h>
#include <stdio.h>
#include <string.h>

#include "../../include/vgh.h"
#include "conv_tiles.h"

typedef __attribute__((ext_vector_type(8))) __bf16 bf16x8_t;
typedef __attribute__((ext_vector_type(4))) __bf16 bf16x4_t;
typedef __attribute__((ext_vector_type(16))) float f32x16_t;
typedef __attribute__((ext_vector_type(4))) float f32x4_t;
typedef __attribute__((ext_vector_type(2))) float f32x2_t;

void vgh_set_error(const char* fmt, ...);

#define VGH_HIP(expr)                                                                       \
    do {                                                                                    \
        hipError_t _e = (expr);                                                             \
        if (_e != hipSuccess) {                                                             \
            vgh_set_error("%s:%d: %s -> %s", __FILE__, __LINE__, #expr, hipGetErrorString(_e)); \
            return VGH_ERR_HIP;                                                             \
        }                                                                                   \
    } while (0)

#define VGH_REQUIRE(cond, ...)            \
    do {                                  \
        if (!(cond)) {                    \
            vgh_set_error(__VA_ARGS__);   \
            return VGH_ERR_INVALID;       \
        }                                 \
    } while (0)

#define VGH_TRACE_TILES 16
#define VGH_TRACE_MARKS 4

#ifdef VGH_EXPERIMENTS
#define VGH_ABLATE(a, bit) ((a).ablate & (bit))
#define VGH_MARK(a, tile_no, k)                                                                                                      \
    do {                                                                                                                             \
        if ((a).trace && threadIdx.x == 0 && (tile_no) < VGH_TRACE_TILES)                                                            \
            (a).trace[((size_t)blockIdx.x * VGH_TRACE_TILES + (tile_no)) * VGH_TRACE_MARKS + (k)] = __builtin_amdgcn_s_memtime();   \
    } while (0)
#define VGH_MARK_BLOCK(a, k)                                                                                                  \
    do {                                                                                                                      \
        if ((a).trace && threadIdx.x == 0 && blockIdx.x < 8192)                                                               \
            (a).trace[((size_t)blockIdx.x * VGH_TRACE_TILES) * VGH_TRACE_MARKS + (k)] = __builtin_amdgcn_s_memtime();        \
    } while (0)
struct VghMarkAtExit {
    unsigned long long* t;
    __device__ ~VghMarkAtExit() {
        if (t && threadIdx.x == 0 && blockIdx.x < 8192) t[((size_t)blockIdx.x * VGH_TRACE_TILES) * VGH_TRACE_MARKS + 3] = __builtin_amdgcn_s_memtime();
    }
};
#define VGH_MARK_EXIT(a) VghMarkAtExit vgh_mark_at_exit_{(a).trace}
#else
#define VGH_ABLATE(a, bit) 0
#define VGH_MARK(a, tile_no, k) \
    do {                        \
    } while (0)
#define VGH_MARK_BLOCK(a, k) \
    do {                     \
    } while (0)
#define VGH_MARK_EXIT(a) \
    do {                 \
    } while (0)
#endif

int vgh_nms_select(const float* boxes_dev, const float* scores_dev, const float* flame_dev, int B, int n_in, float conf_thr, float iou_thr, int keep_k,
                   int32_t* keep_idx_dev, int32_t* counts_dev, float* out_boxes_dev, float* out_scores_dev, float* out_flame_dev, int capacity, int32_t* head_row_dev,
                   int32_t* head_image_dev, int32_t* n_heads_dev, int32_t* ticket_dev, const vgh_head_level* lazy_levels, int n_levels, const int32_t* lazy_idx_dev,
                   int shape_c, int expr_c, void* stream);
int vgh_launch_conv(const ConvArgs& a, int force_cfg, hipStream_t stream);
#define VGH_TILE_LAUNCHER(name) int name(const ConvArgs& a, const TileGrid& g, int lds, hipStream_t st)
int vgh_launch_conv_b2b(const ConvArgs& a, hipStream_t stream);
int vgh_launch_conv_ds_b2b(const ConvArgs& a, hipStream_t stream);
int vgh_launch_conv_ds(const ConvArgs& a, const TileGrid& g, hipStream_t stream);
int vgh_launch_conv_w(const ConvArgs& a, const TileGrid& g, hipStream_t stream);
int vgh_launch_stem_ds_b2b(const ConvArgs& a, const void* image_u8, int Hi, int Wi, const float* wstem, const float* bstem, hipStream_t stream);
int vgh_launch_conv_split(const ConvArgs& a, int force_cfg, hipStream_t stream);
void vgh_pack_conv_weights_split_host(const float* w, int cout_pad, int ksize, int cin, int fmt, uint16_t* dst, float* out_scale);
uint8_t vgh_f32_to_e4m3_host(float f);
void vgh_pack_conv_weights_fp8_host(const float* w, int cout_pad, int ksize, int cin, uint8_t* dst, float* wscale);
void vgh_pack_conv_weights_i8_host(const float* w, int cout_pad, int ksize, int cin, uint8_t* dst, float* wscale);
int vgh_launch_conv_pp(const ConvArgs& a, TileFamily family, int bc, const TileGrid& g, int max_blocks_per_xcd, hipStream_t stream);
int vgh_conv_pp_lds(int bc);
int vgh_conv_max_blocks_per_xcd();
int vgh_conv_persistent_blocks_per_xcd(const ConvArgs& a, int chunk, int blocks_per_cu);
int vgh_conv_pick_cfg(const ConvArgs& a);
int vgh_conv_cfg_ok_for(int cfg, const ConvArgs& a);
int vgh_conv_prepare(ConvArgs& a);
int vgh_conv_pick_auto(const ConvArgs& a);
int vgh_conv_split_pick(const ConvArgs& a);
void vgh_pack_conv_weights_host(const float* w, int cout_pad, int ksize, int cin, uint16_t* dst);
template <class Src, class Cvt>
static inline void vgh_pack_conv_image(const Src* w, int cout_pad, int ksize, int cin, uint16_t* dst, Cvt cvt) {
    const int cblocks = cin / 32, taps = ksize * ksize;
    for (int tap = 0; tap < taps; ++tap)
        for (int cb = 0; cb < cblocks; ++cb) {
            const int kb = tap * cblocks + cb;
            for (int co = 0; co < cout_pad; ++co) {
                const Src* src = w + ((size_t)co * taps + tap) * cin + cb * 32;
                uint16_t* d = dst + ((size_t)kb * cout_pad + co) * 32;
                const int sw = (co >> 2) & 3;
                for (int chunk = 0; chunk < 4; ++chunk) {
                    const int slot = chunk ^ sw;
                    for (int e = 0; e < 8; ++e) d[slot * 8 + e] = cvt(src[chunk * 8 + e]);
                }
            }
        }
}
static inline size_t vgh_wpack_elems(int cout_pad, int ksize, int cin) { return (size_t)cout_pad * ksize * ksize * cin; }

static inline void vgh_fastdiv_magic(unsigned d, unsigned* m, unsigned* s) {
    unsigned sh = 0;
    while ((1ull << sh) < d) ++sh;
    *m = (unsigned)((((1ull << 32) * ((1ull << sh) - d)) / d) + 1);
    *s = sh;
}

static inline uint16_t vgh_f32_to_bf16_host(float f) {
    uint32_t u;
    memcpy(&u, &f, 4);
    if ((u & 0x7fffffffu) > 0x7f800000u) return (uint16_t)((u >> 16) | 0x40);
    u += 0x7fffu + ((u >> 16) & 1u);
    return (uint16_t)(u >> 16);
}

int vgh_launch_stem(const void* image, int image_fmt, int B, int H, int W, const float* w ,
                    const float* bias , uint16_t* out, int64_t out_pitch, int out_coff, int store_ch , int fmt, int plane,
                    hipStream_t stream);
int vgh_launch_stem_ds(const void* image, int image_fmt, int B, int H, int W, const float* wstem, const float* bstem, const uint16_t* wds, const float* bds, uint16_t* out,
                       int64_t out_pitch, int out_coff, hipStream_t stream);
void vgh_pack_stem_ds_weights_host(const float* w , uint16_t* dst );
int vgh_launch_conv_f32(const ConvArgs& a, const float* wdense, hipStream_t stream);
int vgh_launch_stem_f32(const void* image, int image_fmt, int B, int H, int W, const float* w, const float* bias, float* out, int64_t out_pitch, int out_coff,
                        hipStream_t stream);
int vgh_launch_spp_pool_f32(float* buf, int64_t pitch, int coff, int C, int B, int H, int W, hipStream_t stream);
int vgh_launch_spp_pool(uint16_t* buf, int64_t pitch, int coff, int C, int B, int H, int W, int fmt, int plane, hipStream_t stream);

int vgh_stream_acquire_internal(int device, const hipStream_t* avoid, int n_avoid, hipStream_t* out, bool low_priority = false);
void vgh_stream_release_internal(int device, hipStream_t s, bool low_priority = false);
struct vgh_net;
int vgh_net_lane_streams(vgh_net* n, hipStream_t main, hipStream_t* out);
extern "C" __attribute__((visibility("hidden"))) int vgh_net_device(vgh_net* n);
extern "C" __attribute__((visibility("hidden"))) int vgh_net_set_pred_guard(vgh_net* n, void* event);
extern "C" __attribute__((visibility("hidden"))) uint64_t vgh_net_generation(vgh_net* n);

struct vgh_lb_batch;
int vgh_lb_prepare(vgh_lb_batch** lb, int S, int max_batch, int arena_batch, int image_fmt, const void* imgs, int B);
int vgh_lb_chunk(vgh_lb_batch* lb, int chunk, int n, hipStream_t stream);
int vgh_lb_unpad_read(vgh_lb_batch* lb, hipStream_t stream);
uint8_t* vgh_lb_canvas(const vgh_lb_batch* lb);
float* vgh_lb_unpad(const vgh_lb_batch* lb);
void vgh_lb_destroy(vgh_lb_batch* lb);
```

### head_detector_amd/engine.py

```python
from __future__ import annotations

import ctypes as C
import json
import os
from dataclasses import dataclass
from typing import Dict, List, Optional, Tuple

import numpy as np
import torch

from . import _lib, arch
from .flame import FLAMELayer

TUNING_DIR = os.path.join(os.path.dirname(os.path.abspath(__file__)), "tuning")


@dataclass
class Detections:

    boxes: torch.Tensor
    scores: torch.Tensor
    flame_params: torch.Tensor
    counts: torch.Tensor
    n_heads: Optional[torch.Tensor] = None
    head_image_cap: Optional[torch.Tensor] = None
    vertices_cap: Optional[torch.Tensor] = None
    rpy_cap: Optional[torch.Tensor] = None
    _n: Optional[int] = None

    @property
    def num_heads(self) -> int:
        if self._n is None:
            self._n = int(self.n_heads.item()) if self.n_heads is not None else 0
        return self._n

    @property
    def head_image(self) -> Optional[torch.Tensor]:
        return None if self.head_image_cap is None else self.head_image_cap[: self.num_heads].long()

    @property
    def vertices_3d(self) -> Optional[torch.Tensor]:
        return None if self.vertices_cap is None else self.vertices_cap[: self.num_heads]

    @property
    def head_pose(self) -> Optional[torch.Tensor]:
        return None if self.rpy_cap is None else self.rpy_cap[: self.num_heads]


def _alias(ptr: int, shape, typestr: str, device: torch.device) -> torch.Tensor:

    class _Ext:
        pass

    e = _Ext()
    e.__cuda_array_interface__ = dict(shape=tuple(shape), typestr=typestr, data=(int(ptr), False), version=2)
    return torch.as_tensor(e, device=device)


class VGHeadsEngine:
    def __init__(self, variant: str = "vgg_heads_l", state_dict: Optional[Dict[str, np.ndarray]] = None, image_size: int = 640, max_batch: int = 1,
                 device: Optional[int] = None, seed: int = 1, pre_nms_top_k: int = 1000, keep_top_k: int = 100, use_tuning: bool = True,
                 arena_batch: Optional[int] = None, precision: str = "bf16", fp8_scales: Optional[Dict[str, float]] = None, calib_images: Optional[torch.Tensor] = None,
                 fp8_min_px: int = 40, latency_lanes: bool = True):
        if variant not in arch.VARIANTS:
            raise ValueError(f"unknown model variant {variant!r}; known: {sorted(arch.VARIANTS)}")
        if not torch.cuda.is_available():
            raise _lib.VghError("VGHeadsEngine needs a GPU: the HIP path is the only implementation (no CPU fallback)")
        self.lib = _lib.load()
        self.variant, self.image_size, self.max_batch = variant, image_size, max_batch
        self.device_index = torch.cuda.current_device() if device is None else int(device)
        self.device = torch.device("cuda", self.device_index)
        if state_dict is None:
            state_dict = arch.random_state_dict(variant, seed)
        self.precision = precision
        self.fp8_scales = None
        if precision in arch.Q8_PRECISIONS:
            if fp8_scales is None:
                if calib_images is None:
                    import warnings

                    warnings.warn(f"VGHeadsEngine(precision={precision!r}) without fp8_scales / calib_images: the 8-bit link scales are calibrated on two seeded RANDOM "
                                  "images -- adequate for the synthetic benchmark, not for real weights and photographs (pass calib_images or fp8_scales)", stacklevel=2)
                    calib_images = torch.randint(0, 256, (2, image_size, image_size, 3), dtype=torch.uint8, generator=torch.Generator().manual_seed(12345)).to(torch.device("cuda", self.device_index))
                fp8_scales = calibrate_fp8(variant, state_dict, image_size, calib_images, self.device_index, fp8_min_px)
            self.fp8_scales = dict(fp8_scales)
        self.program = arch.build_program(variant, state_dict, image_size, precision, fp8_scales=self.fp8_scales, fp8_min_px=fp8_min_px)
        if max_batch <= LATENCY_MAX_BATCH and latency_lanes:
            arch.schedule_latency(self.program)
        P = self.program
        per_image = max(bf["h"] * bf["w"] * bf["pitch"] * arch.FMT_BYTES[bf["is_f32"]] for bf in P.bufs)
        self.arena_batch = max(1, min(max_batch, ((1 << 31) - 1) // per_image, arena_batch or max_batch))
        w, b = P.arrays()
        bufs = (_lib.BufDesc * len(P.bufs))(*[_lib.BufDesc(bf["h"], bf["w"], bf["pitch"], bf["is_f32"], float(bf.get("scale", 0.0))) for bf in P.bufs])
        fields = [f for f, _ in _lib.OpDesc._fields_]
        ops = (_lib.OpDesc * len(P.ops))(*[_lib.OpDesc(**{f: (op.get(f, 0) if f != "in_buf" else max(op[f], 0)) for f in fields}) for op in P.ops])
        h = C.c_void_p()
        with torch.cuda.device(self.device):
            _lib.check(self.lib.vgh_net_create(self.device_index, image_size, self.arena_batch, bufs, len(P.bufs), ops, len(P.ops), _lib.ptr(w), w.size, _lib.ptr(b), b.size, C.byref(h)))
        self._net = h
        if int(self.lib.vgh_net_b2b_pairs(h)) != len(arch.b2b_pairs(P)):
            raise _lib.VghError(f"back-to-back pairs: the library found {int(self.lib.vgh_net_b2b_pairs(h))}, arch.b2b_pairs {len(arch.b2b_pairs(P))}")
        self.stream = torch.cuda.Stream(device=self.device)
        self.A = sum(lv["h"] * lv["w"] for lv in P.levels)
        self.pre_k, self.keep_k = min(pre_nms_top_k, self.A), keep_top_k
        B, A, k, kk = max_batch, self.A, self.pre_k, keep_top_k
        f32 = dict(dtype=torch.float32, device=self.device)
        i32 = dict(dtype=torch.int32, device=self.device)
        cfg = _lib.DetectCfg()
        cfg.n_levels = len(P.levels)
        for i, lv in enumerate(P.levels):
            cfg.level_buf[i], cfg.level_h[i], cfg.level_w[i], cfg.level_pitch[i], cfg.level_stride[i] = lv["buf"], lv["h"], lv["w"], lv["pitch"], lv["stride"]
        cfg.shape_live, cfg.expr_live, cfg.pre_k, cfg.keep_k, cfg.max_batch = P.shape_c, P.expr_c, k, kk, B
        d = C.c_void_p()
        with torch.cuda.device(self.device):
            _lib.check(self.lib.vgh_detector_create(self._net, None, C.byref(cfg), C.byref(d)))
        self._det = d
        self._flame_ref = None
        pb, ps, pf = C.c_void_p(), C.c_void_p(), C.c_void_p()
        _lib.check(self.lib.vgh_detector_candidate_buffers(self._det, C.byref(pb), C.byref(ps), C.byref(pf)))
        self.cand_boxes = _alias(pb.value, (B, k, 4), "<f4", self.device)
        self.cand_scores = _alias(ps.value, (B, k), "<f4", self.device)
        self.cand_flame = _alias(pf.value, (B, k, _lib.NUM_FLAME_PARAMS), "<f4", self.device)
        sc = lambda which: self.lib.vgh_detector_scratch(self._det, which)
        self.boxes_all = _alias(sc(_lib.SCRATCH_BOXES_ALL), (B, A, 4), "<f4", self.device)
        self.scores_all = _alias(sc(_lib.SCRATCH_SCORES_ALL), (B, A), "<f4", self.device)
        self.idx = _alias(sc(_lib.SCRATCH_TOPK_IDX), (B, k), "<i4", self.device)
        self.keep_idx = _alias(sc(_lib.SCRATCH_KEEP_IDX), (B, kk), "<i4", self.device)
        self.counts = torch.empty(B, **i32)
        self.out_boxes = torch.empty(B, kk, 4, **f32)
        self.out_scores = torch.empty(B, kk, **f32)
        self.out_flame = torch.empty(B, kk, _lib.NUM_FLAME_PARAMS, **f32)
        self.n_heads = torch.zeros(1, **i32)
        self._head_out = None
        self._levels = None
        self._graph_key = None
        self._use_tuning = bool(use_tuning and precision in ("bf16", "fp8", "int8", "fp16", "fp16x3", "bf16x3"))
        self.nsplit = 1
        if self._use_tuning:
            self.load_tuning()

    def close(self):
        if getattr(self, "_det", None) is not None:
            self.lib.vgh_detector_destroy(self._det)
            self._det = None
        if getattr(self, "_net", None) is not None:
            self.lib.vgh_net_destroy(self._net)
            self._net = None

    def __del__(self):
        try:
            self.close()
        except Exception:
            pass

    @property
    def flops_per_image(self) -> float:
        return self.program.flops

    def _sp(self) -> int:
        return self.stream.cuda_stream

    def _levels_arr(self, B: int):
        P = self.program
        arr = (_lib.HeadLevel * len(P.levels))()
        for i, lv in enumerate(P.levels):
            arr[i] = _lib.HeadLevel(self.lib.vgh_net_buffer(self._net, lv["buf"]), lv["h"], lv["w"], lv["pitch"], lv["stride"])
        return arr

    def buffer(self, name_or_id, B: int) -> torch.Tensor:
        P = self.program
        bid = name_or_id if isinstance(name_or_id, int) else next(i for i, bf in enumerate(P.bufs) if bf["name"] == name_or_id)
        bf = P.bufs[bid]
        fmt = bf["is_f32"]
        n = B * bf["h"] * bf["w"] * bf["pitch"]
        self.stream.synchronize()
        if fmt == arch.FMT_FP8:
            t = _alias(self.lib.vgh_net_buffer(self._net, bid), (n,), "|u1", self.device).clone().view(torch.float8_e4m3fn).float() * bf["scale"]
            return t.view(B, bf["h"], bf["w"], bf["pitch"])
        if fmt == arch.FMT_I8:
            t = _alias(self.lib.vgh_net_buffer(self._net, bid), (n,), "|i1", self.device).clone().float() * bf["scale"]
            return t.view(B, bf["h"], bf["w"], bf["pitch"])
        if fmt in (arch.FMT_BF16X2, arch.FMT_F16X2):
            t = _alias(self.lib.vgh_net_buffer(self._net, bid), (2 * n,), "<i2", self.device).clone().view(B, bf["h"], bf["w"], 2, bf["pitch"])
            t = t.view(torch.bfloat16 if fmt == arch.FMT_BF16X2 else torch.float16).float()
            return t[..., 0, :] + t[..., 1, :] * (1.0 if fmt == arch.FMT_BF16X2 else 1.0 / 2048.0)
        t = _alias(self.lib.vgh_net_buffer(self._net, bid), (n,), "<f4" if fmt == arch.FMT_F32 else "<i2", self.device)
        if fmt == arch.FMT_BF16:
            t = t.view(torch.bfloat16)
        elif fmt == arch.FMT_F16:
            t = t.view(torch.float16)
        return t.clone().view(B, bf["h"], bf["w"], bf["pitch"])

    def _check_images(self, images: torch.Tensor) -> Tuple[int, int]:
        S = self.image_size
        if images.dtype == torch.float32 and images.dim() == 4 and images.shape[1:] == (3, S, S):
            fmt = _lib.VGH_IMG_F32_NCHW
        elif images.dtype == torch.uint8 and images.dim() == 4 and images.shape[1:] == (S, S, 3):
            fmt = _lib.VGH_IMG_U8_NHWC
        else:
            raise ValueError(f"images must be f32 [B,3,{S},{S}] or u8 [B,{S},{S},3]; got {images.dtype} {tuple(images.shape)}")
        if not images.is_cuda or not images.is_contiguous():
            raise ValueError("images must be a contiguous GPU tensor")
        B = images.shape[0]
        if B > self.max_batch:
            raise ValueError(f"batch {B} exceeds max_batch {self.max_batch}")
        return B, fmt

    def _images_arg(self, images) -> Tuple[int, int, int]:
        if isinstance(images, torch.Tensor):
            B, fmt = self._check_images(images)
            return B, fmt, images.data_ptr()
        from .video import YUV420Frame

        B = len(images)
        if not 1 <= B <= self.max_batch:
            raise ValueError(f"raw image batch of {B} outside 1..max_batch={self.max_batch}")
        n_frames = sum(isinstance(t, YUV420Frame) for t in images)
        if n_frames:
            if n_frames != B:
                raise ValueError(f"a batch holds YUV420Frames or RGB tensors, not both ({n_frames} of {B} are frames): one call has one image format; convert with frame.to_rgb()")
            arr = (_lib.Yuv420Image * B)()
            for i, f in enumerate(images):
                if f.device != self.device:
                    raise ValueError(f"frame {i}: its planes are on {f.device}, the engine is on {self.device}")
                h, w, _ = f.shape
                arr[i] = _lib.Yuv420Image(f.y.data_ptr(), f.u.data_ptr(), f.v.data_ptr(), h, w, f.y_pitch, f.uv_pitch, f.chroma_step, *f.coefficients)
                for t in f.planes:
                    t.record_stream(self.stream)
            self._raw_arg = arr
            return B, _lib.VGH_IMG_YUV420_RAW, C.addressof(arr)
        arr = (_lib.RawImage * B)()
        for i, t in enumerate(images):
            if not isinstance(t, torch.Tensor) or t.dtype != torch.uint8 or t.dim() != 3 or t.shape[2] < 3 or t.device != self.device:
                raise ValueError(f"raw image {i}: expected a uint8 tensor [h, w, C >= 3] on {self.device}; got {getattr(t, 'dtype', type(t))} {tuple(getattr(t, 'shape', ()))}")
            if t.stride(2) != 1 or t.stride(1) != t.shape[2]:
                raise ValueError(f"raw image {i}: the pixels of a row must be dense (strides (pitch, C, 1)); got {t.stride()}")
            arr[i] = _lib.RawImage(t.data_ptr(), t.shape[0], t.shape[1], t.shape[2], t.stride(0))
            t.record_stream(self.stream)
        self._raw_arg = arr
        return B, _lib.VGH_IMG_U8_RAW, C.addressof(arr)

    def raw_unpad(self) -> Optional[torch.Tensor]:
        p = self.lib.vgh_detector_scratch(self._det, _lib.SCRATCH_UNPAD)
        return None if not p else _alias(p, (self.max_batch, 3), "<f4", self.device)

    def raw_canvas(self) -> Optional[torch.Tensor]:
        p = self.lib.vgh_detector_scratch(self._det, _lib.SCRATCH_CANVAS)
        S = self.image_size
        return None if not p else _alias(p, (self.arena_batch, S, S, 3), "|u1", self.device)

    def forward_net(self, images: torch.Tensor, use_graph: bool = False) -> int:
        B, fmt = self._check_images(images)
        if B > self.arena_batch:
            raise ValueError(f"forward_net handles at most arena_batch={self.arena_batch} images; use forward_candidates() for larger batches")
        self.stream.wait_stream(torch.cuda.current_stream(self.device))
        if use_graph:
            if getattr(self, "_overlap", False):
                raise ValueError("hipGraph replay cannot honour the prediction-buffer guard of overlap mode: use one or the other")
            key = (images.data_ptr(), B, fmt)
            if self._graph_key != key:
                _lib.check(self.lib.vgh_net_forward(self._net, images.data_ptr(), fmt, B, self._sp()))
                self.stream.synchronize()
                _lib.check(self.lib.vgh_net_capture(self._net, images.data_ptr(), fmt, B, self._sp()))
                self._graph_key = key
            _lib.check(self.lib.vgh_net_forward_graph(self._net, self._sp()))
        else:
            _lib.check(self.lib.vgh_net_forward(self._net, images.data_ptr(), fmt, B, self._sp()))
        return B

    def set_split(self, nsplit: int = 1):
        _lib.check(self.lib.vgh_net_set_split(self._net, int(nsplit)))
        self.nsplit = int(nsplit)
        if self._use_tuning:
            self.load_tuning()

    def set_b2b(self, enable=True):
        _lib.check(self.lib.vgh_net_set_b2b(self._net, int(enable) if enable in (2, 3) and enable is not True else int(bool(enable))))
        self._graph_key = None

    @property
    def stem_fused(self) -> bool:
        return bool(self.lib.vgh_net_stem_fused(self._net))

    @property
    def b2b_pairs(self) -> int:
        return int(self.lib.vgh_net_b2b_pairs(self._net))

    def set_fuse_stem(self, enable: bool = True):
        if not hasattr(self.lib, "vgh_net_set_fuse_stem"):
            raise _lib.VghError("set_fuse_stem: the fused stem + downsample kernel exists in the -DVGH_EXPERIMENTS build only (python -m head_detector_amd.build --experiments)")
        _lib.check(self.lib.vgh_net_set_fuse_stem(self._net, int(bool(enable))))
        self._graph_key = None

    def set_overlap(self, enable: bool = True):
        _lib.check(self.lib.vgh_detector_set_overlap(self._det, int(bool(enable))))
        self._overlap = bool(enable)

    def tune_overlap(self, images: torch.Tensor, flame=None, forwards: int = 8, confidence_threshold: float = 0.5) -> Dict[str, float]:
        import time

        B = int(images.shape[0])
        unpad = torch.tensor([[0.0, 0.0, 1.0]], device=self.device).expand(B, 3).contiguous()

        def run(n):
            for _ in range(n):
                self.forward_net(images)
                self.candidates(B)
                self.select(B, confidence_threshold=confidence_threshold, iou_threshold=0.5, flame=flame, unpad=unpad)
            self.join()
            torch.cuda.synchronize(self.device)

        out = {}
        for on in (True, False):
            self.join()
            self.set_overlap(on)
            run(2)
            t = time.perf_counter()
            run(forwards)
            out["overlapped" if on else "serial"] = (time.perf_counter() - t) / forwards * 1e3
        self.set_overlap(out["overlapped"] <= out["serial"])
        return out

    def join(self):
        _lib.check(self.lib.vgh_detector_join(self._det, self._sp()))
        torch.cuda.current_stream(self.device).wait_stream(self.stream)

    def candidates(self, B: int, at: int = 0, lazy_flame: bool = False):
        self._set_lazy_flame(lazy_flame)
        _lib.check(self.lib.vgh_detector_decode_candidates(self._det, B, at, self._sp()))

    def _set_lazy_flame(self, enable: bool):
        if getattr(self, "_lazy_flame", False) != bool(enable):
            _lib.check(self.lib.vgh_detector_set_lazy_flame(self._det, int(bool(enable))))
            self._lazy_flame = bool(enable)

    def forward_candidates(self, images: torch.Tensor, use_graph: bool = False, lazy_flame: bool = False) -> int:
        self.stream.wait_stream(torch.cuda.current_stream(self.device))
        B, fmt, ptr = self._images_arg(images)
        if use_graph and B <= self.arena_batch and fmt not in _lib.RAW_FORMATS:
            self.forward_net(images, True)
            self.candidates(B, lazy_flame=lazy_flame)
            return B
        self._set_lazy_flame(lazy_flame)
        _lib.check(self.lib.vgh_detector_candidates(self._det, ptr, fmt, B, self._sp()))
        return B

    def _join_if_overlap(self):
        if getattr(self, "_overlap", False):
            _lib.check(self.lib.vgh_detector_join(self._det, self._sp()))

    def model(self, images: torch.Tensor, use_graph: bool = False, copy: bool = True):
        B = self.forward_candidates(images, use_graph)
        self._join_if_overlap()
        torch.cuda.current_stream(self.device).wait_stream(self.stream)
        out = self.cand_boxes[:B], self.cand_scores[:B].unsqueeze(-1), self.cand_flame[:B]
        return tuple(t.clone() for t in out) if copy else out

    def new_output_slot(self, flame: Optional[FLAMELayer] = None, batch: Optional[int] = None) -> Dict[str, torch.Tensor]:
        B, kk = batch or self.max_batch, self.keep_k
        f32 = dict(dtype=torch.float32, device=self.device)
        i32 = dict(dtype=torch.int32, device=self.device)
        nb, ns, nf = B * kk * 4, (B * kk + 3) // 4 * 4, B * kk * _lib.NUM_FLAME_PARAMS
        nf4, nc = (nf + 3) // 4 * 4, (B + 3) // 4 * 4
        flat = torch.zeros(nb + ns + nf4 + nc + 4, **f32)
        ints = flat.view(torch.int32)
        slot = dict(boxes=flat[:nb].view(B, kk, 4), scores=flat[nb:nb + B * kk].view(B, kk), flame=flat[nb + ns:nb + ns + nf].view(B, kk, _lib.NUM_FLAME_PARAMS),
                    counts=ints[nb + ns + nf4:nb + ns + nf4 + B], n_heads=ints[nb + ns + nf4 + nc:nb + ns + nf4 + nc + 1])
        if flame is not None:
            cap = min(B * self.keep_k, flame.max_heads)
            slot.update(cap=cap, head_image=torch.empty(cap, **i32), proj=torch.empty(cap, flame.num_vertices, 3, **f32), rpy=torch.empty(cap, 3, **f32))
        return slot

    def _detect_out(self, B: int, flame: Optional[FLAMELayer], unpad: Optional[torch.Tensor], n_heads_out: Optional[torch.Tensor] = None,
                    slot: Optional[Dict[str, torch.Tensor]] = None) -> Tuple["_lib.DetectOut", Detections]:
        o = _lib.DetectOut()
        ob, os_, of, oc = (slot["boxes"], slot["scores"], slot["flame"], slot["counts"]) if slot is not None else (self.out_boxes, self.out_scores, self.out_flame, self.counts)
        o.boxes_dev, o.scores_dev, o.flame_dev, o.counts_dev = ob.data_ptr(), os_.data_ptr(), of.data_ptr(), oc.data_ptr()
        det = Detections(ob[:B], os_[:B], of[:B], oc[:B])
        if flame is not None:
            handle = flame._need_handle()
            if self._flame_ref is not flame:
                _lib.check(self.lib.vgh_detector_set_flame(self._det, handle))
                self._flame_ref = flame
            if slot is not None:
                if "proj" not in slot or slot["proj"].shape[1] != flame.num_vertices:
                    raise ValueError("output slot was created without (or for another) FLAME layer: new_output_slot(flame)")
                cap, himg, proj, rpy = slot["cap"], slot["head_image"], slot["proj"], slot["rpy"]
            else:
                cap = min(self.max_batch * self.keep_k, flame.max_heads)
                if self._head_out is None or self._head_out[0] != cap or self._head_out[2].shape[1] != flame.num_vertices:
                    self._head_out = (cap, torch.empty(cap, dtype=torch.int32, device=self.device), torch.empty(cap, flame.num_vertices, 3, dtype=torch.float32, device=self.device),
                                      torch.empty(cap, 3, dtype=torch.float32, device=self.device))
                cap, himg, proj, rpy = self._head_out
            if unpad is not None:
                if unpad.shape != (B, 3) or unpad.dtype != torch.float32 or not unpad.is_cuda or not unpad.is_contiguous():
                    raise ValueError("unpad must be a contiguous float32 GPU tensor [B,3] = (pad_x, pad_y, scale) per image")
                o.unpad_dev = unpad.data_ptr()
            nh = n_heads_out if n_heads_out is not None else (slot["n_heads"] if slot is not None else self.n_heads)
            o.n_heads_dev, o.head_image_dev, o.head_capacity = nh.data_ptr(), himg.data_ptr(), cap
            o.proj_dev, o.rpy_dev = proj.data_ptr(), rpy.data_ptr()
            det.n_heads, det.head_image_cap, det.vertices_cap, det.rpy_cap = nh, himg, proj, rpy
        return o, det

    def detect(self, images, confidence_threshold: float = 0.5, iou_threshold: float = 0.5, flame: Optional[FLAMELayer] = None,
               unpad: Optional[torch.Tensor] = None, use_graph: bool = False, reuse_outputs: bool = False) -> Detections:
        cur = torch.cuda.current_stream(self.device)
        self.stream.wait_stream(cur)
        B, fmt, ptr = self._images_arg(images)
        net_first = not getattr(self, "_overlap", False)
        slot = None
        if not net_first and not reuse_outputs:
            with torch.cuda.stream(self.stream):
                slot = self.new_output_slot(flame, B)
        if use_graph and B <= self.arena_batch and fmt not in _lib.RAW_FORMATS:
            self.forward_candidates(images, True, lazy_flame=True)
        else:
            self._set_lazy_flame(True)
            _lib.check(self.lib.vgh_detector_candidates(self._det, ptr, fmt, B, self._sp()))
        if net_first and not reuse_outputs:
            with torch.cuda.stream(self.stream):
                slot = self.new_output_slot(flame, B)
        o, det = self._detect_out(B, flame, unpad, None, slot)
        _lib.check(self.lib.vgh_detector_select(self._det, B, float(confidence_threshold), float(iou_threshold), C.byref(o), self._sp()))
        if getattr(self, "_overlap", False):
            _lib.check(self.lib.vgh_detector_join(self._det, self._sp()))
        cur.wait_stream(self.stream)
        if slot is not None:
            for t in slot.values():
                if isinstance(t, torch.Tensor):
                    t.record_stream(cur)
        return det

    def select(self, B: int, confidence_threshold: float = 0.5, iou_threshold: float = 0.5, flame: Optional[FLAMELayer] = None,
               unpad: Optional[torch.Tensor] = None, n_heads_out: Optional[torch.Tensor] = None, slot: Optional[Dict[str, torch.Tensor]] = None) -> Detections:
        o, det = self._detect_out(B, flame, unpad, n_heads_out, slot)
        _lib.check(self.lib.vgh_detector_select(self._det, B, float(confidence_threshold), float(iou_threshold), C.byref(o), self._sp()))
        return det

    def streams_in_use(self) -> List["torch.cuda.Stream"]:
        out = (C.c_void_p * 4)()
        _lib.check(self.lib.vgh_detector_streams(self._det, self._sp(), out))
        ptrs = [out[i] for i in range(max(self.nsplit - 1, 0))] + ([out[3]] if out[3] else [])
        return [self.stream] + [torch.cuda.ExternalStream(p, device=self.device) for p in ptrs]

    def acquire_stream(self) -> "torch.cuda.Stream":
        out = (C.c_void_p * 4)()
        _lib.check(self.lib.vgh_detector_streams(self._det, self._sp(), out))
        lanes, side = [out[i] for i in range(3)], out[3]
        order = [self._sp()] + lanes[: max(self.nsplit - 1, 0)] + ([side] if side else []) + lanes[max(self.nsplit - 1, 0):]
        avoid = (C.c_void_p * len(order))(*order)
        got = C.c_void_p()
        _lib.check(self.lib.vgh_stream_acquire(self.device.index or 0, avoid, len(order), C.byref(got)))
        return torch.cuda.ExternalStream(got.value, device=self.device)

    def make_event(self) -> "torch.cuda.Event":
        return torch.cuda.Event()

    def record_select_done(self, event: "torch.cuda.Event"):
        if not event.cuda_event:
            event.record(self.stream)
        _lib.check(self.lib.vgh_detector_record(self._det, event.cuda_event, self._sp()))

    def join_into(self, stream: "torch.cuda.Stream"):
        _lib.check(self.lib.vgh_detector_join(self._det, stream.cuda_stream))

    def profile_ops(self, images: torch.Tensor, repeats: int = 1) -> List[dict]:
        B, fmt = self._check_images(images)
        self.stream.wait_stream(torch.cuda.current_stream(self.device))
        passes = []
        for _ in range(max(1, repeats)):
            ms = (C.c_float * len(self.program.ops))()
            _lib.check(self.lib.vgh_net_profile(self._net, images.data_ptr(), fmt, B, self._sp(), ms))
            passes.append(list(ms))
        med = [sorted(col)[len(col) // 2] for col in zip(*passes)]
        out = []
        for op, t in zip(self.program.ops, med):
            fl = 2.0 * op["macs"] * B
            by = arch.op_algorithmic_bytes(self.program, op, B)
            out.append(dict(name=op["name"], kind=op["kind"], ms=float(t), gflop=fl / 1e9, tflops=(fl / (t * 1e-3) / 1e12) if t > 0 else 0.0, gemm=op["gemm"],
                            read_mb=by["read"] / 1e6, write_mb=by["write"] / 1e6, gbps=((by["read"] + by["write"]) / (t * 1e-3) / 1e9) if t > 0 else 0.0))
        return out

    def set_cfg(self, op_index: int, cfg: int):
        _lib.check(self.lib.vgh_net_set_cfg(self._net, op_index, cfg))
        self._graph_key = None

    def cfg_names(self) -> List[str]:
        return tile_names(self.lib, self.precision)

    def op_tiles(self) -> Dict[int, str]:
        names = self.cfg_names()
        out = {}
        for i in range(len(self.program.ops)):
            c = int(self.lib.vgh_net_op_cfg(self._net, i))
            if c >= 0:
                out[i] = names[c]
        return out

    def cfg_ok(self, cfg: int, op: dict) -> bool:
        return tile_can_run(self.lib, self.program, self.precision, cfg, op)

    def load_tuning(self, path: Optional[str] = None) -> int:
        if path is not None:
            self._tuning_path = path
        path = getattr(self, "_tuning_path", None) or os.path.join(TUNING_DIR, "conv_cfg.json")
        if not os.path.exists(path):
            return 0
        table = json.load(open(path))
        names = {n: i for i, n in enumerate(self.cfg_names())}
        applied = 0
        for i, op in enumerate(self.program.ops):
            if op["kind"] != 1 or arch.op_touches_fp8(self.program, op):
                continue
            pre = "" if self.precision in ("bf16", "fp8", "int8") else self.precision + ":"
            name = tuning_lookup(table, op, self.max_batch, getattr(self, "nsplit", 1), pre)
            if name in names and self.cfg_ok(names[name], op):
                self.set_cfg(i, names[name])
                applied += 1
            else:
                self.set_cfg(i, -1)
        return applied


def tile_names(lib, precision: str) -> List[str]:
    if precision in ("fp16x3", "bf16x3", "fp16"):
        return [lib.vgh_conv_split_cfg_name(i).decode() for i in range(lib.vgh_conv_split_num_cfgs())]
    return [lib.vgh_conv_cfg_name(i).decode() for i in range(lib.vgh_conv_num_cfgs())]


def tile_can_run(lib, program: "arch.Program", precision: str, cfg: int, op: dict) -> bool:
    names = tile_names(lib, precision)
    ob = program.bufs[op["out_buf"]]
    al = all(op[k] % 8 == 0 for k in ("out_coff", "out_coff2", "out_split", "cout_store", "res_coff")) and ob["pitch"] % 8 == 0
    fast = int(ob["is_f32"] != arch.FMT_F32 and al)
    if precision in ("fp16x3", "bf16x3", "fp16"):
        if precision != "fp16" and names[cfg][0] == "g":
            return False
        return bool(lib.vgh_conv_split_cfg_ok(cfg, op["ksize"], op["stride"], op["cout_pad"], fast, op["shuffle"], op.get("grp_cout", 0)))
    if not lib.vgh_conv_cfg_ok(cfg, op["ksize"], op["stride"], op["cout_pad"], fast, op["shuffle"]):
        return False
    if names[cfg].startswith("t") and (op.get("res_buf", -1) >= 0 or op.get("grp_cout") or op.get("act") == 2):
        return False
    if names[cfg][0] in "ghs" and (op.get("grp_cout") or op.get("act") == 2):
        return False
    return not op.get("grp_cout") or op["grp_cout"] % lib.vgh_conv_cfg_cout_tile(cfg) == 0


def calibrate_fp8(variant: str, state_dict: Optional[Dict[str, np.ndarray]], image_size: int, images: torch.Tensor, device: Optional[int] = None, fp8_min_px: int = 40) -> Dict[str, float]:
    n = int(images.shape[0])
    if n == 0:
        raise ValueError("calibrate_fp8: no calibration image")
    chunk = min(n, CALIB_CHUNK)
    eng = VGHeadsEngine(variant, state_dict, image_size, max_batch=chunk, device=device, precision="bf16", use_tuning=False)
    try:
        links = arch.fp8_link_names(variant, image_size, fp8_min_px)
        out = {link: 0.0 for link in links}
        for at in range(0, n, chunk):
            x = images[at:at + chunk].contiguous()
            for a0 in range(0, x.shape[0], eng.arena_batch):
                xa = x[a0:a0 + eng.arena_batch].contiguous()
                eng.forward_net(xa)
                eng.stream.synchronize()
                for link, (src, live) in links.items():
                    out[link] = max(out[link], float(eng.buffer(src, xa.shape[0])[..., :live].float().abs().max()))
        return out
    finally:
        eng.close()


CALIB_CHUNK = 8
LATENCY_MAX_BATCH = 2


def _epilogue_class(op: dict) -> str:
    return "_f32" if op.get("out_f32") else "_sh" if op.get("shuffle") else ""


def tuning_key(op: dict, batch: int, nsplit: int = 1, bucket: Optional[int] = None, res: Optional[bool] = None, cls: Optional[str] = None) -> str:
    m, n, k = op["gemm"]
    if bucket is None:
        bucket = 1 if batch <= 2 else (8 if batch <= 16 else (32 if batch <= 32 else 64))
    lanes = f"x{nsplit}" if nsplit > 1 else ""
    grp = f"_g{op['grp_cout']}" if op.get("grp_cout") else ""
    rs = "_res" if (op.get("res_buf", -1) >= 0 if res is None else res) else ""
    cl = _epilogue_class(op) if cls is None else cls
    return f"b{bucket}{lanes}_m{m}_n{n}_k{k}_ks{op['ksize']}_s{op['stride']}{grp}{rs}{cl}"


def tuning_lookup(table: Dict[str, str], op: dict, batch: int, nsplit: int = 1, prefix: str = "") -> Optional[str]:
    b32 = batch > 32
    cls = _epilogue_class(op)
    keys = []
    for c in ((None, "") if cls else (None,)):
        for r in ((None, False) if op.get("res_buf", -1) >= 0 else (None,)):
            keys += [tuning_key(op, batch, nsplit, res=r, cls=c)] + ([tuning_key(op, batch, nsplit, bucket=32, res=r, cls=c)] if b32 else [])
            keys += [tuning_key(op, batch, res=r, cls=c)] + ([tuning_key(op, batch, bucket=32, res=r, cls=c)] if b32 else [])
    for k in keys:
        name = table.get(prefix + k)
        if name is None:
            continue
        if cls and not k.endswith(cls) and not prefix and not name[0].isdigit():
            continue
        return name
    return None
```

Before: 5407 images/sec.

## Defer FLAME head 1x1 convs and compute them only for NMS survivor rows

Marks the final 1x1 convs that write the FLAME channels of the prediction buffers as deferrable. When the lazy FLAME gather is on, the forward skips them, and a new survivor_rows kernel recomputes those channels only for the rows kept by NMS from the bf16 input features. Any other reader of the buffers first triggers the deferred convs. This removes most of the dense FLAME-head conv work, since only a few heads per image survive. In exchange it adds deferral bookkeeping, graph-capture interactions and a per-survivor matvec kernel.

```diff
diff --git a/head_detector_amd/csrc/detect.hip b/head_detector_amd/csrc/detect.hip
--- a/head_detector_amd/csrc/detect.hip
+++ b/head_detector_amd/csrc/detect.hip
@@ -22,6 +22,11 @@
     int32_t* head_image = nullptr;
     int32_t* ticket = nullptr;
     bool lazy_flame = false;
+    bool rows_ok = false;
+    bool defer_allowed = true;
+    bool rows_on() const { return rows_ok && defer_allowed; }
+    vgh_row_op row_ops[VGH_MAX_LEVELS * kMaxRowOps] = {};
+    int n_row_ops[VGH_MAX_LEVELS] = {};
     enum : uint8_t { SRC_NONE = 0, SRC_EAGER = 1, SRC_LAZY = 2 };
     std::vector<uint8_t> row_src;
     int lazy_rows = 0;
@@ -119,6 +124,24 @@
         A += cfg->level_h[l] * cfg->level_w[l];
     }
     d->A = A;
+    {
+        const int width = cfg->shape_live + cfg->expr_live + 13;
+        bool ok = true;
+        for (int l = 0; l < cfg->n_levels && ok; ++l) {
+            vgh_row_op* ro = d->row_ops + l * kMaxRowOps;
+            const int k = d->n_row_ops[l] = vgh_net_row_ops(net, cfg->level_buf[l], ro, kMaxRowOps);
+            ok = k >= 1;
+            int stored = 0;
+            for (int i = 0; i < k && ok; ++i) {
+                ok = vgh_row_op_ok(ro[i], width);
+                stored += ro[i].cout_store;
+                for (int j = 0; j < i && ok; ++j)
+                    ok = ro[i].out_coff + ro[i].cout_store <= ro[j].out_coff || ro[j].out_coff + ro[j].cout_store <= ro[i].out_coff;
+            }
+            ok = ok && stored == width;
+        }
+        d->rows_ok = ok;
+    }
     d->row_src.assign((size_t)cfg->max_batch, vgh_detector::SRC_NONE);
     if (cfg->pre_k > A) {
         delete d;
@@ -207,12 +230,15 @@
     const vgh_detect_cfg& c = d->cfg;
     vgh_head_level lv[VGH_MAX_LEVELS];
     for (int l = 0; l < c.n_levels; ++l) {
-        lv[l].pred_dev = (const float*)vgh_net_buffer(d->net, c.level_buf[l]);
+        lv[l].pred_dev = (const float*)vgh_net_buffer_ptr(d->net, c.level_buf[l]);
         lv[l].h = c.level_h[l];
         lv[l].w = c.level_w[l];
         lv[l].pitch = c.level_pitch[l];
         lv[l].stride = c.level_stride[l];
     }
+    const bool lazy = d->lazy_flame && at == 0;
+    if (!(lazy && d->rows_on()))
+        if (int rc0 = vgh_net_run_deferred(d->net, stream)) return rc0;
     void* st = stream;
     if (d->overlap) {
         if (int rc0 = ensure_side(d, (hipStream_t)stream)) return rc0;
@@ -226,7 +252,6 @@
     int rc;
     if ((rc = vgh_head_decode(lv, c.n_levels, n, ba, sa, st))) return rc;
     if ((rc = vgh_topk(sa, n, d->A, c.pre_k, ix, d->cand_scores + (size_t)at * c.pre_k, st))) return rc;
-    const bool lazy = d->lazy_flame && at == 0;
     if ((rc = vgh_gather_candidates(lv, c.n_levels, n, d->A, c.shape_live, c.expr_live, ba, ix, c.pre_k, d->cand_boxes + (size_t)at * c.pre_k * 4,
                                     lazy ? nullptr : d->cand_flame + (size_t)at * c.pre_k * VGH_NUM_FLAME_PARAMS, st)))
         return rc;
@@ -297,10 +322,13 @@
                 "buffers no longer hold that batch (queue the select before the next forward, or decode with the lazy FLAME gather off)",
                 (unsigned long long)d->lazy_gen, (unsigned long long)(vgh_net_generation(d->net) - d->lazy_gen));
     VGH_REQUIRE(!lazy || c.keep_k <= 1024, "detector_select: the lazy FLAME gather needs keep_k <= 1024");
+    if (lazy && !d->rows_on())
+        if ((rc = vgh_net_run_deferred(d->net, stream))) return rc;
+    const bool rows = lazy && d->rows_on() && vgh_net_deferred_pending(d->net);
     if (c.keep_k <= 1024) {
         vgh_head_level lv[VGH_MAX_LEVELS];
         for (int l = 0; l < c.n_levels; ++l) {
-            lv[l].pred_dev = (const float*)vgh_net_buffer(d->net, c.level_buf[l]);
+            lv[l].pred_dev = (const float*)vgh_net_buffer_ptr(d->net, c.level_buf[l]);
             lv[l].h = c.level_h[l];
             lv[l].w = c.level_w[l];
             lv[l].pitch = c.level_pitch[l];
@@ -308,8 +336,12 @@
         }
         if ((rc = vgh_nms_select(d->cand_boxes, d->cand_scores, d->cand_flame, B, c.pre_k, conf_thr, iou_thr, c.keep_k, d->keep_idx, o->counts_dev, o->boxes_dev,
                                  o->scores_dev, o->flame_dev, capacity, want_heads ? d->head_row : nullptr, himg, o->n_heads_dev, d->ticket, lazy ? lv : nullptr,
-                                 c.n_levels, lazy ? d->idx : nullptr, c.shape_live, c.expr_live, stream)))
+                                 c.n_levels, lazy ? d->idx : nullptr, c.shape_live, c.expr_live, stream, rows)))
             return rc;
+        if (rows)
+            if ((rc = vgh_survivor_rows(lv, c.n_levels, d->row_ops, d->n_row_ops, B, c.pre_k, c.keep_k, d->idx, d->keep_idx, o->counts_dev, c.shape_live, c.expr_live, o->flame_dev,
+                                        stream)))
+                return rc;
         if (lazy && d->overlap && stream == (void*)d->side) {
             VGH_HIP(hipEventRecord(d->ev_cand, d->side));
         }
@@ -375,7 +407,8 @@
 int vgh_detector_set_lazy_flame(vgh_detector* d, int enable) {
     VGH_REQUIRE(d, "detector_set_lazy_flame: null handle");
     d->lazy_flame = enable != 0;
-    return VGH_OK;
+    d->defer_allowed = enable != 2;
+    return d->rows_ok ? vgh_net_set_defer(d->net, d->lazy_flame && d->defer_allowed) : VGH_OK;
 }
 
 int vgh_detector_streams(vgh_detector* d, void* main_stream, void** out) {
diff --git a/head_detector_amd/csrc/net.hip b/head_detector_amd/csrc/net.hip
--- a/head_detector_amd/csrc/net.hip
+++ b/head_detector_amd/csrc/net.hip
@@ -27,7 +27,7 @@
     uint16_t* wds = nullptr;
     float* gscale = nullptr;
     float* dvec = nullptr;
-    int overhang_ok = 0, b2b = 0;
+    int overhang_ok = 0, b2b = 0, deferrable = 0;
     hipEvent_t ev_done = nullptr;
 };
 
@@ -56,6 +56,11 @@
     int fuse_b2b = 1;
     int stem3_ok = 0;
     uint64_t generation = 0;
+    DeferState defer;
+    bool skipping = false;
+    bool graph_skips = false;
+    int graph_B = 0;
+    hipStream_t last_stream = nullptr;
     int fuse_stem = 0;
 };
 
@@ -136,6 +141,7 @@
         case VGH_OP_CONV: {
             if ((fused || stem3) && op_index == n->stem_pair + 1) return VGH_OK;
             if (n->fuse_b2b && op.b2b == 2) return VGH_OK;
+            if (n->skipping && op.deferrable) return VGH_OK;
             ConvArgs a;
             if (int rc = net_conv_args(n, op, B, at, &a)) return rc;
             a.grid_share = share;
@@ -359,6 +365,7 @@
         op.out_scale = oscale[i];
         op.overhang_ok = po.overhang_ok;
         op.b2b = po.b2b;
+        op.deferrable = po.deferrable;
         if (ops[i].kind == VGH_OP_CONV || ops[i].kind == VGH_OP_STEM) {
             op.wf32 = (float*)(n->wblob + po.w);
             op.bias = (float*)(n->wblob + po.bias);
@@ -416,6 +423,13 @@
     VGH_REQUIRE(B >= 0 && B <= n->max_batch, "net_forward: B=%d exceeds max_batch=%d", B, n->max_batch);
     hipStream_t main = (hipStream_t)stream;
     ++n->generation;
+    n->defer.forward(B, n->defer.skip());
+    n->last_stream = main;
+    struct Skipping {
+        vgh_net* n;
+        ~Skipping() { n->skipping = false; }
+    } skipping{n};
+    n->skipping = n->defer.pending;
     if (int rc = ensure_lanes(n, main)) return rc;
     if (n->nsplit > 1 && B > 1) return net_forward_split(n, image_dev, image_fmt, B, main);
     bool pending[vgh_net::kLanes] = {false, false, false, false}, used[vgh_net::kLanes] = {false, false, false, false};
@@ -461,6 +475,7 @@
     VGH_REQUIRE(B >= 0 && B <= n->max_batch, "net_profile: B=%d exceeds max_batch=%d", B, n->max_batch);
     hipStream_t st = (hipStream_t)stream;
     ++n->generation;
+    n->defer.forward(B, false);
     if (int rc = ensure_lanes(n, st)) return rc;
     const size_t m = n->ops.size();
     struct Events {
@@ -517,6 +532,9 @@
     if (int rc = ensure_lanes(n, st)) return rc;
     VGH_HIP(hipStreamBeginCapture(st, hipStreamCaptureModeThreadLocal));
     int rc = vgh_net_forward(n, image_dev, image_fmt, B, stream);
+    n->graph_skips = n->defer.pending;
+    n->graph_B = B;
+    n->defer.forward(0, false);
     hipError_t e = hipStreamEndCapture(st, &n->graph);
     if (rc) return rc;
     VGH_HIP(e);
@@ -528,11 +546,41 @@
     VGH_REQUIRE(n && n->graph_exec, "net_forward_graph: call vgh_net_capture first");
     VGH_REQUIRE(!n->pred_guard, "net_forward_graph: a prediction guard event is set (detector overlap mode); use vgh_net_forward");
     ++n->generation;
+    n->defer.forward(n->graph_B, n->graph_skips);
+    n->last_stream = (hipStream_t)stream;
     VGH_HIP(hipGraphLaunch(n->graph_exec, (hipStream_t)stream));
     return VGH_OK;
 }
 
-void* vgh_net_buffer(vgh_net* n, int buf_id) { return (n && buf_id >= 0 && buf_id < (int)n->buf_ptr.size()) ? n->buf_ptr[buf_id] : nullptr; }
+int vgh_net_set_defer(vgh_net* n, int on) {
+    VGH_REQUIRE(n, "net_set_defer: null handle");
+    n->defer.on = on != 0;
+    return VGH_OK;
+}
+
+int vgh_net_run_deferred(vgh_net* n, void* stream) {
+    VGH_REQUIRE(n, "net_run_deferred: null handle");
+    const int B = n->defer.take();
+    if (B == 0) return VGH_OK;
+    for (const NetOp& op : n->ops)
+        if (op.deferrable)
+            if (int rc = net_run_op(n, op, nullptr, VGH_IMG_U8_NHWC, B, 0, (hipStream_t)stream)) return rc;
+    return VGH_OK;
+}
+
+int vgh_net_deferred_pending(vgh_net* n) { return n && n->defer.pending ? 1 : 0; }
+
+void* vgh_net_buffer_ptr(vgh_net* n, int buf_id) { return (n && buf_id >= 0 && buf_id < (int)n->buf_ptr.size()) ? n->buf_ptr[buf_id] : nullptr; }
+void* vgh_net_buffer(vgh_net* n, int buf_id) {
+    void* p = vgh_net_buffer_ptr(n, buf_id);
+    if (p && n->defer.pending)
+        for (const NetOp& op : n->ops)
+            if (op.deferrable && op.d.out_buf == buf_id) {
+                if (vgh_net_run_deferred(n, n->last_stream)) return nullptr;
+                break;
+            }
+    return p;
+}
 int64_t vgh_net_buffer_bytes(vgh_net* n, int buf_id) { return (n && buf_id >= 0 && buf_id < (int)n->buf_bytes.size()) ? n->buf_bytes[buf_id] : -1; }
 
 #ifdef VGH_EXPERIMENTS
@@ -580,6 +628,18 @@
 }
 
 uint64_t vgh_net_generation(vgh_net* n) { return n ? n->generation : 0; }
+
+int vgh_net_row_ops(vgh_net* n, int out_buf, vgh_row_op* out, int max_ops) {
+    if (!n || !out) return -1;
+    int k = 0;
+    for (const NetOp& op : n->ops) {
+        if (!op.deferrable || op.d.out_buf != out_buf) continue;
+        if (k == max_ops) return -1;
+        const vgh_buf_desc& ib = n->bufs[op.d.in_buf];
+        out[k++] = vgh_row_op{(const uint16_t*)n->buf_ptr[op.d.in_buf], op.wpack, op.bias, ib.pitch, op.d.in_coff, op.d.cin / 32, op.d.cout_pad, op.d.cout_store, op.d.out_coff, op.d.act};
+    }
+    return k;
+}
 int vgh_net_max_batch(vgh_net* n) { return n ? n->max_batch : 0; }
 int vgh_net_device(vgh_net* n) { return n ? n->device : 0; }
 int vgh_net_image_size(vgh_net* n) { return n ? n->image_size : 0; }
diff --git a/head_detector_amd/csrc/net_plan.h b/head_detector_amd/csrc/net_plan.h
--- a/head_detector_amd/csrc/net_plan.h
+++ b/head_detector_amd/csrc/net_plan.h
@@ -85,6 +85,43 @@
     return true;
 }
 
+inline bool net_op_deferrable(const vgh_buf_desc* bufs, const vgh_op_desc* ops, int n_ops, int i, bool fused_or_awaited) {
+    const vgh_op_desc& d = ops[i];
+    if (d.kind != VGH_OP_CONV || d.ksize != 1 || d.stride != 1 || fused_or_awaited) return false;
+    if (bufs[d.out_buf].is_f32 != VGH_FMT_F32 || bufs[d.in_buf].is_f32 != VGH_FMT_BF16) return false;
+    if (d.res_buf >= 0 || d.shuffle || d.grp_cout || d.act == VGH_ACT_SILU || d.out_coff < VGH_PRED_FLAME_OFF || d.out_split < d.cout_pad || d.cout_store > d.cout_pad) return false;
+    int first_f32 = n_ops;
+    for (int j = n_ops - 1; j >= 0; --j)
+        if (ops[j].kind == VGH_OP_CONV && bufs[ops[j].out_buf].is_f32 == VGH_FMT_F32) first_f32 = j;
+    for (int j = 0; j < n_ops; ++j) {
+        const vgh_op_desc& e = ops[j];
+        if (e.kind == VGH_OP_FORK) continue;
+        const bool conv = e.kind == VGH_OP_CONV;
+        if ((conv || e.kind == VGH_OP_SPP_POOL) && e.in_buf == d.out_buf) return false;
+        if (conv && e.res_buf == d.out_buf) return false;
+        const bool writes_in = (conv || e.kind == VGH_OP_STEM) ? e.out_buf == d.in_buf : e.kind == VGH_OP_SPP_POOL && e.in_buf == d.in_buf;
+        if (writes_in && (j > i || j < first_f32)) return false;
+    }
+    return true;
+}
+
+struct DeferState {
+    bool on = false;
+    bool pending = false;
+    int B = 0;
+    bool skip() const { return on; }
+    void forward(int batch, bool skipped) {
+        pending = skipped;
+        B = skipped ? batch : 0;
+    }
+    int take() {
+        const int b = pending ? B : 0;
+        pending = false;
+        B = 0;
+        return b;
+    }
+};
+
 struct NetPlan {
     std::vector<int64_t> buf_off, buf_bytes;
     int64_t arena_bytes = 0;
@@ -95,6 +132,7 @@
         int b2b = 0;
         int overhang_ok = 0;
         int ev_done = 0;
+        int deferrable = 0;
     };
     std::vector<Op> ops;
     int64_t wds = -1;
@@ -206,6 +244,10 @@
         for (int a = 1; a < kNetLanes; ++a)
             for (int b = 1; b < kNetLanes; ++b) w[a][b] = w[a][b] || (w[a][k] && w[k][b]);
     for (int a = 1; a < kNetLanes; ++a) p->lane_wait_cycle = p->lane_wait_cycle || w[a][a];
+    for (int i = 0; i < n_ops; ++i) {
+        const NetPlan::Op& o = p->ops[i];
+        p->ops[i].deferrable = net_op_deferrable(bufs, ops, n_ops, i, o.b2b || o.ev_done || o.overhang_ok) && ops[i].out_coff + ops[i].cout_store <= bufs[ops[i].out_buf].pitch ? 1 : 0;
+    }
     return VGH_OK;
 #undef PLAN_REQUIRE
 }
diff --git a/head_detector_amd/csrc/postproc.hip b/head_detector_amd/csrc/postproc.hip
--- a/head_detector_amd/csrc/postproc.hip
+++ b/head_detector_amd/csrc/postproc.hip
@@ -177,7 +177,7 @@
 }
 
 __device__ __forceinline__ float flame_channel(const float* __restrict__ pr, int c, int S, int E, int ax, int ay, float st) {
-    const int o_shape = VGH_PRED_FLAME_OFF, o_expr = o_shape + S, o_rot = o_expr + E, o_jaw = o_rot + 6, o_tr = o_jaw + 3, o_sc = o_tr + 3;
+    const int o_shape = 0, o_expr = o_shape + S, o_rot = o_expr + E, o_jaw = o_rot + 6, o_tr = o_jaw + 3, o_sc = o_tr + 3;
     float v = 0.0f;
     if (c < 300) {
         if (c < S) v = tanhf(pr[o_shape + c]) * 3.0f;
@@ -215,7 +215,7 @@
     if (lane < 4) out_boxes[((int64_t)b * k + j) * 4 + lane] = boxes[((int64_t)b * A + a) * 4 + lane];
     if (!out_flame) return;
     float* of = out_flame + ((int64_t)b * k + j) * VGH_NUM_FLAME_PARAMS;
-    for (int c = lane; c < VGH_NUM_FLAME_PARAMS; c += 64) of[c] = flame_channel(pr, c, S, E, ax, ay, st);
+    for (int c = lane; c < VGH_NUM_FLAME_PARAMS; c += 64) of[c] = flame_channel(pr + VGH_PRED_FLAME_OFF, c, S, E, ax, ay, st);
 }
 
 __device__ __forceinline__ bool iou_gt(const float4 a, const float area_a, const float4 b, const float thr) {
@@ -286,7 +286,7 @@
                                                           float conf, float thr, int keep_k, int32_t* __restrict__ keep_idx, int32_t* __restrict__ counts,
                                                           float* __restrict__ ob, float* __restrict__ os, float* __restrict__ of, int B, int capacity,
                                                           int32_t* __restrict__ head_row, int32_t* __restrict__ head_image, int32_t* __restrict__ n_heads,
-                                                          int32_t* __restrict__ ticket, Levels L, const int32_t* __restrict__ lazy_idx, int S, int E) {
+                                                          int32_t* __restrict__ ticket, Levels L, const int32_t* __restrict__ lazy_idx, int S, int E, int rows_later) {
     __shared__ float4 sb[1024];
     __shared__ unsigned long long removed[16];
     __shared__ int s_keep[1024];
@@ -309,7 +309,7 @@
         const int64_t sr = (int64_t)b * n_in + s_keep[j];
         if (lane < 4) ob[o * 4 + lane] = boxes[sr * 4 + lane];
         if (lane == 0) os[o] = scores[sr];
-        if (of) {
+        if (of && !rows_later) {
             if (lazy_idx) {
                 const int a = lazy_idx[sr];
                 const int l = find_level(L, a);
@@ -317,7 +317,7 @@
                 const float* pr = L.pred[l] + ((int64_t)b * (L.h[l] * L.w[l]) + p) * L.pitch[l];
                 const int ay = p / L.w[l], ax = p - ay * L.w[l];
                 const float st = (float)L.stride[l];
-                for (int c = lane; c < VGH_NUM_FLAME_PARAMS; c += 64) of[o * VGH_NUM_FLAME_PARAMS + c] = flame_channel(pr, c, S, E, ax, ay, st);
+                for (int c = lane; c < VGH_NUM_FLAME_PARAMS; c += 64) of[o * VGH_NUM_FLAME_PARAMS + c] = flame_channel(pr + VGH_PRED_FLAME_OFF, c, S, E, ax, ay, st);
             } else {
                 for (int c = lane; c < VGH_NUM_FLAME_PARAMS; c += 64) of[o * VGH_NUM_FLAME_PARAMS + c] = flame[sr * VGH_NUM_FLAME_PARAMS + c];
             }
@@ -404,6 +404,84 @@
     if (lane == 0) os[o] = sorted_scores[(int64_t)b * k + pos];
     if (of)
         for (int c = lane; c < flame_w; c += 64) of[o * flame_w + c] = flame[s * flame_w + c];
+}
+
+struct RowOps {
+    Levels L;
+    vgh_row_op op[MAX_LEVELS][kMaxRowOps];
+    int n[MAX_LEVELS];
+};
+constexpr int ROW_W = 416;
+
+__global__ __launch_bounds__(256) void survivor_rows_kernel(const RowOps R, int n_in, int keep_k, const int32_t* __restrict__ idx, const int32_t* __restrict__ keep_idx,
+                                                            const int32_t* __restrict__ counts, int S, int E, float* __restrict__ out) {
+    __shared__ float rows[32][ROW_W];
+    const int b = blockIdx.y, j0 = blockIdx.x * 32, tid = threadIdx.x, lane = tid & 63, w = tid >> 6;
+    const int kept = min(max(counts[b], 0), keep_k);
+    if (j0 >= kept) return;
+    for (int i = tid; i < 32 * ROW_W; i += 256) (&rows[0][0])[i] = 0.0f;
+    const Levels& L = R.L;
+    const int A = L.start[L.n];
+    const int px = lane & 31, hi = lane >> 5;
+    const bool valid = j0 + px < kept;
+    int lvl = -1, p = 0;
+    if (valid) {
+        const int pos = min(max(keep_idx[(int64_t)b * keep_k + j0 + px], 0), n_in - 1);
+        const int a = min(max(idx[(int64_t)b * n_in + pos], 0), A - 1);
+        lvl = find_level(L, a);
+        p = a - L.start[lvl];
+    }
+    __syncthreads();
+    for (int l = 0; l < L.n; ++l) {
+        const bool mine = lvl == l;
+        if (!__any(mine)) continue;
+        const int hw = L.h[l] * L.w[l];
+        int units = 0;
+        for (int k = 0; k < R.n[l]; ++k) units += R.op[l][k].cout_pad >> 5;
+        for (int u = w; u < units; u += 4) {
+            int k = 0, t = u;
+            while (t >= (R.op[l][k].cout_pad >> 5)) t -= R.op[l][k++].cout_pad >> 5;
+            const vgh_row_op& o = R.op[l][k];
+            const int co = t * 32 + px;
+            const uint16_t* const xr = o.in + ((int64_t)b * hw + p) * o.in_pitch + o.in_coff + hi * 8;
+            const uint16_t* const wr = o.wpack + (int64_t)co * 32;
+            const int sw = (co >> 2) & 3;
+            f32x16_t acc;
+#pragma unroll
+            for (int r = 0; r < 16; ++r) acc[r] = 0.0f;
+            for (int kb = 0; kb < o.cblocks; ++kb) {
+#pragma unroll
+                for (int h = 0; h < 2; ++h) {
+                    const bf16x8_t af = *(const bf16x8_t*)(wr + (int64_t)kb * o.cout_pad * 32 + ((2 * h + hi) ^ sw) * 8);
+                    bf16x8_t bf;
+#pragma unroll
+                    for (int e = 0; e < 8; ++e) bf[e] = (__bf16)0.0f;
+                    if (mine) bf = *(const bf16x8_t*)(xr + kb * 32 + h * 16);
+                    acc = __builtin_amdgcn_mfma_f32_32x32x16_bf16(af, bf, acc, 0, 0, 0);
+                }
+            }
+            const float act_lo = o.act == VGH_ACT_RELU ? 0.0f : __builtin_nanf("");
+            const int oc = o.out_coff - VGH_PRED_FLAME_OFF;
+#pragma unroll
+            for (int q = 0; q < 4; ++q)
+#pragma unroll
+                for (int e = 0; e < 4; ++e) {
+                    const int c = t * 32 + q * 8 + hi * 4 + e;
+                    if (mine && c < o.cout_store) rows[px][oc + c] = fmaxf(acc[q * 4 + e] + o.bias[c], act_lo);
+                }
+        }
+    }
+    __syncthreads();
+    for (int r = w; r < 32 && j0 + r < kept; r += 4) {
+        const int pos = min(max(keep_idx[(int64_t)b * keep_k + j0 + r], 0), n_in - 1);
+        const int a = min(max(idx[(int64_t)b * n_in + pos], 0), A - 1);
+        const int l = find_level(L, a);
+        const int pp = a - L.start[l];
+        const int ay = pp / L.w[l], ax = pp - ay * L.w[l];
+        const float st = (float)L.stride[l];
+        const int64_t o = (int64_t)b * keep_k + j0 + r;
+        for (int c = lane; c < VGH_NUM_FLAME_PARAMS; c += 64) out[o * VGH_NUM_FLAME_PARAMS + c] = flame_channel(rows[r], c, S, E, ax, ay, st);
+    }
 }
 
 int make_levels(const vgh_head_level* levels, int n_levels, Levels* L) {
@@ -489,7 +567,7 @@
 int vgh_nms_select(const float* boxes_dev, const float* scores_dev, const float* flame_dev, int B, int n_in, float conf_thr, float iou_thr, int keep_k,
                    int32_t* keep_idx_dev, int32_t* counts_dev, float* out_boxes_dev, float* out_scores_dev, float* out_flame_dev, int capacity, int32_t* head_row_dev,
                    int32_t* head_image_dev, int32_t* n_heads_dev, int32_t* ticket_dev, const vgh_head_level* lazy_levels, int n_levels, const int32_t* lazy_idx_dev,
-                   int shape_c, int expr_c, void* stream) {
+                   int shape_c, int expr_c, void* stream, int rows_later) {
     VGH_REQUIRE(n_in >= 0 && n_in <= 1024 && keep_k >= 1 && keep_k <= 1024, "nms_select: n_in=%d / keep_k=%d must be <= 1024", n_in, keep_k);
     VGH_REQUIRE(!head_row_dev || (head_image_dev && n_heads_dev && ticket_dev), "nms_select: the head list needs head_image, n_heads and the ticket");
     if (B == 0) return VGH_OK;
@@ -501,7 +579,32 @@
     }
     hipLaunchKernelGGL(nms_select_kernel, dim3(B), dim3(1024), 0, (hipStream_t)stream, boxes_dev, scores_dev, flame_dev, n_in, conf_thr, iou_thr, keep_k, keep_idx_dev,
                        counts_dev, out_boxes_dev, out_scores_dev, out_flame_dev, B, capacity, head_row_dev, head_image_dev, n_heads_dev, ticket_dev, L, lazy_idx_dev, shape_c,
-                       expr_c);
+                       expr_c, rows_later);
+    VGH_HIP(hipGetLastError());
+    return VGH_OK;
+}
+
+int vgh_survivor_rows(const vgh_head_level* levels, int n_levels, const vgh_row_op* ops, const int* n_ops, int B, int n_in, int keep_k, const int32_t* idx_dev,
+                      const int32_t* keep_idx_dev, const int32_t* counts_dev, int shape_c, int expr_c, float* out_dev, void* stream) {
+    VGH_REQUIRE(levels && ops && n_ops && idx_dev && keep_idx_dev && counts_dev && out_dev, "survivor_rows: null argument");
+    VGH_REQUIRE(n_in >= 1 && keep_k >= 1 && keep_k <= n_in, "survivor_rows: n_in=%d / keep_k=%d", n_in, keep_k);
+    VGH_REQUIRE(shape_c >= 0 && shape_c <= 300 && expr_c >= 0 && expr_c <= 100, "survivor_rows: bad live channel counts");
+    RowOps R;
+    memset(&R, 0, sizeof(R));
+    if (int rc = make_levels(levels, n_levels, &R.L)) return rc;
+    const int width = shape_c + expr_c + 13;
+    for (int l = 0; l < n_levels; ++l) {
+        VGH_REQUIRE(n_ops[l] >= 1 && n_ops[l] <= kMaxRowOps, "survivor_rows: level %d has %d ops", l, n_ops[l]);
+        R.n[l] = n_ops[l];
+        for (int k = 0; k < n_ops[l]; ++k) {
+            const vgh_row_op& o = ops[l * kMaxRowOps + k];
+            VGH_REQUIRE(vgh_row_op_ok(o, width), "survivor_rows: level %d op %d does not write FLAME channels of the prediction row from 16-byte aligned bf16 rows", l, k);
+            R.op[l][k] = o;
+        }
+    }
+    if (B == 0) return VGH_OK;
+    hipLaunchKernelGGL(survivor_rows_kernel, dim3((keep_k + 31) / 32, B), dim3(256), 0, (hipStream_t)stream, R, n_in, keep_k, idx_dev, keep_idx_dev, counts_dev, shape_c, expr_c,
+                       out_dev);
     VGH_HIP(hipGetLastError());
     return VGH_OK;
 }
diff --git a/head_detector_amd/csrc/vgh_internal.h b/head_detector_amd/csrc/vgh_internal.h
--- a/head_detector_amd/csrc/vgh_internal.h
+++ b/head_detector_amd/csrc/vgh_internal.h
@@ -70,7 +70,8 @@
 int vgh_nms_select(const float* boxes_dev, const float* scores_dev, const float* flame_dev, int B, int n_in, float conf_thr, float iou_thr, int keep_k,
                    int32_t* keep_idx_dev, int32_t* counts_dev, float* out_boxes_dev, float* out_scores_dev, float* out_flame_dev, int capacity, int32_t* head_row_dev,
                    int32_t* head_image_dev, int32_t* n_heads_dev, int32_t* ticket_dev, const vgh_head_level* lazy_levels, int n_levels, const int32_t* lazy_idx_dev,
-                   int shape_c, int expr_c, void* stream);
+                   int shape_c, int expr_c, void* stream,
+                   int rows_later = 0);
 int vgh_launch_conv(const ConvArgs& a, int force_cfg, hipStream_t stream);
 #define VGH_TILE_LAUNCHER(name) int name(const ConvArgs& a, const TileGrid& g, int lds, hipStream_t st)
 int vgh_launch_conv_b2b(const ConvArgs& a, hipStream_t stream);
@@ -146,6 +147,24 @@
 extern "C" __attribute__((visibility("hidden"))) int vgh_net_device(vgh_net* n);
 extern "C" __attribute__((visibility("hidden"))) int vgh_net_set_pred_guard(vgh_net* n, void* event);
 extern "C" __attribute__((visibility("hidden"))) uint64_t vgh_net_generation(vgh_net* n);
+struct vgh_row_op {
+    const uint16_t* in;
+    const uint16_t* wpack;
+    const float* bias;
+    int in_pitch, in_coff, cblocks, cout_pad, cout_store, out_coff, act;
+};
+constexpr int kMaxRowOps = 4;
+extern "C" __attribute__((visibility("hidden"))) int vgh_net_set_defer(vgh_net* n, int on);
+extern "C" __attribute__((visibility("hidden"))) int vgh_net_run_deferred(vgh_net* n, void* stream);
+extern "C" __attribute__((visibility("hidden"))) int vgh_net_deferred_pending(vgh_net* n);
+extern "C" __attribute__((visibility("hidden"))) void* vgh_net_buffer_ptr(vgh_net* n, int buf_id);
+static inline bool vgh_row_op_ok(const vgh_row_op& o, int width) {
+    return o.in && o.wpack && o.bias && o.cblocks >= 1 && o.cout_pad >= 32 && o.cout_pad % 32 == 0 && o.cout_store >= 1 && o.cout_store <= o.cout_pad && o.in_coff >= 0 && o.in_coff % 8 == 0 &&
+           o.in_pitch % 8 == 0 && o.in_coff + 32 * o.cblocks <= o.in_pitch && o.out_coff >= VGH_PRED_FLAME_OFF && o.out_coff - VGH_PRED_FLAME_OFF + o.cout_store <= width && o.act != VGH_ACT_SILU;
+}
+extern "C" __attribute__((visibility("hidden"))) int vgh_net_row_ops(vgh_net* n, int out_buf, vgh_row_op* out, int max_ops);
+int vgh_survivor_rows(const vgh_head_level* levels, int n_levels, const vgh_row_op* ops , const int* n_ops, int B, int n_in, int keep_k,
+                      const int32_t* idx_dev, const int32_t* keep_idx_dev, const int32_t* counts_dev, int shape_c, int expr_c, float* out_dev, void* stream);
 
 struct vgh_lb_batch;
 int vgh_lb_prepare(vgh_lb_batch** lb, int S, int max_batch, int arena_batch, int image_fmt, const void* imgs, int B);
diff --git a/head_detector_amd/engine.py b/head_detector_amd/engine.py
--- a/head_detector_amd/engine.py
+++ b/head_detector_amd/engine.py
@@ -173,6 +173,7 @@
         bf = P.bufs[bid]
         fmt = bf["is_f32"]
         n = B * bf["h"] * bf["w"] * bf["pitch"]
+        self.lib.vgh_net_buffer(self._net, bid)
         self.stream.synchronize()
         if fmt == arch.FMT_FP8:
             t = _alias(self.lib.vgh_net_buffer(self._net, bid), (n,), "|u1", self.device).clone().view(torch.float8_e4m3fn).float() * bf["scale"]
@@ -257,7 +258,7 @@
         if use_graph:
             if getattr(self, "_overlap", False):
                 raise ValueError("hipGraph replay cannot honour the prediction-buffer guard of overlap mode: use one or the other")
-            key = (images.data_ptr(), B, fmt)
+            key = (images.data_ptr(), B, fmt, getattr(self, "_lazy_flame", False))
             if self._graph_key != key:
                 _lib.check(self.lib.vgh_net_forward(self._net, images.data_ptr(), fmt, B, self._sp()))
                 self.stream.synchronize()
@@ -331,8 +332,15 @@
 
     def _set_lazy_flame(self, enable: bool):
         if getattr(self, "_lazy_flame", False) != bool(enable):
-            _lib.check(self.lib.vgh_detector_set_lazy_flame(self._det, int(bool(enable))))
+            _lib.check(self.lib.vgh_detector_set_lazy_flame(self._det, (1 if getattr(self, "_defer_allowed", True) else 2) if enable else 0))
             self._lazy_flame = bool(enable)
+
+    def set_defer(self, allow: bool = True):
+        self._defer_allowed = bool(allow)
+        lazy = getattr(self, "_lazy_flame", False)
+        self._lazy_flame = None
+        self._set_lazy_flame(lazy)
+        self._graph_key = None
 
     def forward_candidates(self, images: torch.Tensor, use_graph: bool = False, lazy_flame: bool = False) -> int:
         self.stream.wait_stream(torch.cuda.current_stream(self.device))
```

Measured after the change: 5567 images/sec (median of 6 runs). +3.0%, better.
